# dordanino12/unet-convlstm

Hardware: AMD Instinct MI355X
Metric: training frames/sec, Moving-MNIST 64x64 seq-20 (higher is better)
Workload: dtype bf16; 1 GPU; TemporalUNetDualView(base_ch=64, use_skip_lstm=True) train step, 64x64 seq-20, per-GPU batch 32, AdamW+clip; global_batch=32, seq_len=20, parallelism=dp1

## Files before the change

include/uclstm.h:

```cpp
#ifndef UCLSTM_H
#define UCLSTM_H

#include <stdint.h>

#ifdef __cplusplus
extern "C" {
#endif

#define UCLSTM_ABI_VERSION 16

#define UCLSTM_OK            0
#define UCLSTM_E_BADARG     -1
#define UCLSTM_E_LAUNCH     -2
#define UCLSTM_E_NODEVICE   -3

#define UCLSTM_ACT_TYPE_BF16 0
#define UCLSTM_ACT_TYPE_F16  1


typedef struct {
    const void* ptr;
    int32_t C;
    int32_t Hs, Ws;
    int32_t offY, offX;
} uclstm_src;

typedef struct {
    void* ptr;
    int32_t n_begin, n_end;
    int32_t C, c_off;
    int32_t Hd, Wd;
    int32_t scale, oy, ox;
} uclstm_seg;

#define UCLSTM_EPI_STORE 0
#define UCLSTM_EPI_LSTM  1
#define UCLSTM_EPI_ATOMIC 2

typedef struct {
    int32_t n_img, H, W, groups;
    int32_t ktap, scale, pad;
    int32_t nsrc;
    uclstm_src src[2];
    const void* wp;
    int32_t N, Ktot;
    const float* bias;
    const float* col_scale;
    const float* col_shift;
    int32_t relu;
    int32_t epi;
    int32_t nseg;
    uclstm_seg seg[4];
    float* stats;
    int32_t Hd_p;
    const float* c_prev;
    float* c_out;
    void* h_out;
    void* gates_out;
    const float* pre_add;
    float* acc_out;
    int32_t acc_ld;
    int32_t ksplit;
    int64_t acc_slab;
} uclstm_igemm_desc;

int32_t uclstm_igemm_tiles_per_group(int32_t n_img, int32_t H, int32_t W, int32_t groups, int32_t N);

int32_t uclstm_igemm_fwd(const uclstm_igemm_desc* d, void* stream);
int32_t uclstm_igemm_fwd_shape(const uclstm_igemm_desc* desc);
int32_t uclstm_igemm_ksplit_used(int32_t Ktot, int32_t ktap, int32_t ksplit);

int32_t uclstm_igemm_fwd_group(const uclstm_igemm_desc* descs, int32_t n, void* stream);
int32_t uclstm_igemm_fwd_group_blocks(const uclstm_igemm_desc* descs, int32_t n);

int32_t uclstm_igemm_fwd_group_tap(const uclstm_igemm_desc* descs, int32_t n, void* stream);
int32_t uclstm_igemm_fwd_group_tap_blocks(const uclstm_igemm_desc* descs, int32_t n);

typedef struct {
    int32_t n_img, H, W;
    int32_t ktap, scale, pad;
    int32_t nsrc;
    uclstm_src src[2];
    int32_t N, Ktot;
    int32_t nseg;
    uclstm_seg seg[4];
    float* dwp;
    int32_t splits;
    int32_t accumulate;
    int32_t overlapped;
    int32_t reserved_;
    int64_t slab;
} uclstm_wgrad_desc;
int32_t uclstm_igemm_wgrad(const uclstm_wgrad_desc* d, void* stream);
int32_t uclstm_igemm_wgrad_splits(const uclstm_wgrad_desc* d);
int32_t uclstm_igemm_wgrad_shape(const uclstm_wgrad_desc* d);

#define UCLSTM_NMODE_IDENTITY 0
#define UCLSTM_NMODE_LSTM     1
#define UCLSTM_NMODE_TAPMAJOR 2
#define UCLSTM_KMODE_IDENTITY 0
#define UCLSTM_KMODE_GATES    1
#define UCLSTM_KMODE_IM2COL   2

typedef struct {
    int32_t N, Ktot;
    int32_t taps, nsrc;
    int32_t kseg[2], cvalid[2], choff[2];
    int32_t n_mode, n_valid, n_cp;
    int32_t k_mode, k_hdp, k_hd;
    int32_t tap_flip;
    int64_t stride_n, stride_k, stride_tap, stride_ntap;
} uclstm_pack_desc;

int32_t uclstm_pack_weights(const uclstm_pack_desc* d, const float* w, void* wp, void* stream);
typedef struct {
    uclstm_pack_desc d;
    const float* w;
    void* wp;
    int32_t block0, nblocks, gx, family;
    uint32_t div[15];
    int32_t pad_;
} uclstm_pack_job;
int32_t uclstm_pack_job_init(uclstm_pack_job* job , const uclstm_pack_desc* d, const float* w, void* wp, int32_t block0);
int32_t uclstm_pack_weights_batched(const uclstm_pack_job* jobs_dev ,
                                    int32_t njobs, int32_t family, int32_t total_blocks, void* stream);

int32_t uclstm_unpack_wgrad(const uclstm_pack_desc* d, const float* dwp, int32_t nslab ,
                            int64_t slab , float* grad, int32_t accumulate, void* stream);
int32_t uclstm_unpack_wgrad_ordered_groups(const uclstm_pack_desc* d, int32_t nslab);
int32_t uclstm_unpack_wgrad_ordered(const uclstm_pack_desc* d, const float* dwp, int32_t nslab, int64_t slab, float* scratch,
                                    float* grad, int32_t accumulate, void* stream);
int32_t uclstm_pack_bias(const uclstm_pack_desc* d, const float* b, float* bp, void* stream);

int32_t uclstm_bn_finalize(float* stats, int32_t groups, int32_t tiles_per_group, int32_t Cp, int32_t C,
                           int64_t count_per_group, const float* gamma, const float* beta,
                           float* running_mean, float* running_var, float momentum, float eps,
                           float* scale, float* shift, float* mean, float* rstd, void* stream);
int32_t uclstm_bn_stats_fwd(float* stats, int32_t groups, int32_t tiles_per_group, int32_t Cp, int32_t C, int64_t count_per_group,
                            const float* gamma, const float* beta, float eps, float* scale, float* shift, float* mean, float* rstd,
                            void* stream);
int32_t uclstm_bn_running_stats(const float* stats, int32_t groups, int32_t tiles_per_group, int32_t Cp, int32_t C,
                                int64_t count_per_group, float* running_mean, float* running_var, float momentum, void* stream);

int32_t uclstm_bn_stats_partial(const float* stats, int32_t groups, int32_t tiles_per_group, int32_t Cp, double* sums64, void* stream);
int32_t uclstm_bn_stats_from_sums(const double* sums64, int64_t world_count_per_group, float* stats, int32_t groups,
                                  int32_t tiles_per_group, int32_t Cp, int32_t C, const float* gamma, const float* beta, float eps,
                                  float* scale, float* shift, float* mean, float* rstd, void* stream);
int32_t uclstm_bn_bwd_sums_stage(const float* sums, double* sums64, int64_t n, void* stream);
int32_t uclstm_bn_bwd_sums_finish(const double* sums64, double inv_world, float* sums_dz, int64_t n, void* stream);

int32_t uclstm_bn_apply_relu(const void* z, void* a, const float* scale, const float* shift,
                             int64_t pixels, int64_t pixels_per_group, int32_t Cp, void* stream);
int64_t uclstm_bn_bwd_reduce_rows(int64_t pixels, int64_t pixels_per_group);
int32_t uclstm_bn_bwd_reduce(const void* z, const void* da, const float* scale, const float* shift,
                             const float* mean, const float* rstd, float* partials, float* sums,
                             int64_t pixels, int64_t pixels_per_group, int32_t Cp, void* stream);
int32_t uclstm_bn_bwd_apply(const void* z, const void* da, const float* scale, const float* shift,
                            const float* mean, const float* rstd, const float* sums, void* dz,
                            int64_t pixels, int64_t pixels_per_group, int32_t Cp, void* stream);

int64_t uclstm_bn_pool_bwd_rows(int64_t n_img, int32_t H, int32_t W, int32_t Cp, int32_t groups);
int32_t uclstm_bn_apply_relu_pool(const void* z, void* a, void* p, const float* scale, const float* shift, int64_t n_img, int32_t H,
                                  int32_t W, int32_t Cp, int32_t groups, void* stream);
int32_t uclstm_bn_pool_bwd_reduce(const void* z, const void* dskip, const void* dp, const float* scale, const float* shift,
                                  const float* mean, const float* rstd, float* partials, float* sums, int64_t n_img, int32_t H,
                                  int32_t W, int32_t Cp, int32_t groups, void* stream);
int32_t uclstm_bn_pool_bwd_apply(const void* z, const void* dskip, const void* dp, const float* scale, const float* shift,
                                 const float* mean, const float* rstd, const float* sums, void* dz, int64_t n_img, int32_t H,
                                 int32_t W, int32_t Cp, int32_t groups, void* stream);

int32_t uclstm_bn_head_fwd(const void* z, const float* scale, const float* shift, const float* w, const float* b, float* y,
                           int64_t pixels, int64_t pixels_per_group, int32_t Cp, int32_t C, void* stream);
int32_t uclstm_bn_head_bwd_reduce(const void* z, const float* dy, const float* scale, const float* shift, const float* mean,
                                  const float* rstd, const float* w, float* partials, float* sums, float* dw, float* db,
                                  int64_t pixels, int64_t pixels_per_group, int32_t Cp, int32_t C, void* stream);
int32_t uclstm_bn_head_bwd_apply(const void* z, const float* dy, const float* scale, const float* shift, const float* mean,
                                 const float* rstd, const float* sums, const float* w, void* dz, int64_t pixels,
                                 int64_t pixels_per_group, int32_t Cp, int32_t C, void* stream);

int32_t uclstm_bn_head_bwd_reduce_ordered(const void* z, const float* dy, const float* scale, const float* shift, const float* mean,
                                          const float* rstd, const float* w, float* partials, float* head_partials, float* sums,
                                          float* dw, float* db, int64_t pixels, int64_t pixels_per_group, int32_t Cp, int32_t C,
                                          int32_t act_type, void* stream);

int32_t uclstm_bn_bwd_param_grads(const float* sums, int32_t groups, int32_t Cp, int32_t C, float* dgamma, float* dbeta,
                                  int32_t accumulate, void* stream);

int32_t uclstm_maxpool2_fwd(const void* a, void* p, int32_t n_img, int32_t H, int32_t W, int32_t Cp, void* stream);
int32_t uclstm_maxpool2_bwd(const void* a, const void* dp, const void* add, void* da, int32_t n_img, int32_t H, int32_t W, int32_t Cp,
                            void* stream);

int32_t uclstm_splitk_finish(const float* pre, int32_t nslab, int64_t slab, int32_t ld, const float* bias, const float* col_scale,
                             const float* col_shift, int32_t relu, void* out, int64_t pixels, int32_t C, void* stream);

int32_t uclstm_lstm_bwd_pointwise(const void* gates, const float* c_prev, const float* c_new,
                                  const void* dh_a, const void* dh_b, int32_t dh_b_is_f32 ,
                                  int32_t dh_b_nslab , int64_t dh_b_slab ,
                                  float* dc_io, int32_t dc_is_zero, void* dgates, int64_t pixels, int32_t Hd_p, void* stream);
int32_t uclstm_lstm_fwd_pointwise(float* pre, int32_t nslab ,
                                  int64_t slab ,
                                  int32_t clear ,
                                  const float* pre_add ,
                                  const float* bias, const float* c_prev, float* c_out, void* h_out,
                                  void* gates_out, int64_t pixels, int32_t Hd_p, void* stream);
typedef struct {
    float* pre;
    const float* pre_add;
    const float* bias;
    const float* c_prev;
    float* c_out;
    void* h_out;
    void* gates_out;
    int64_t slab;
    int64_t pixels;
    int32_t nslab, clear, Hd_p, reserved_;
} uclstm_lstm_fwd_pw_args;
int32_t uclstm_lstm_fwd_pointwise_group(const uclstm_lstm_fwd_pw_args* args, int32_t n, void* stream);

int32_t uclstm_nchw_to_nhwc(const float* x, void* out, int32_t n_img, int32_t C, int32_t Cp, int32_t H, int32_t W,
                            int32_t inner, int64_t inner_stride, int64_t outer_stride, void* stream);
int32_t uclstm_nhwc_to_nchw(const void* a, float* out, int32_t n_img, int32_t C, int32_t Cp, int32_t H, int32_t W, void* stream);
int32_t uclstm_nchw_grad_to_nhwc(const float* g, void* out, int32_t n_img, int32_t C, int32_t Cp, int32_t H, int32_t W, void* stream);
int32_t uclstm_im2col3x3_first(const float* x, void* out, int32_t n_img, int32_t C, int32_t Kp, int32_t H, int32_t W,
                               int32_t inner, int64_t inner_stride, int64_t outer_stride, void* stream);
int32_t uclstm_nchw_to_nhwc_f32(const float* x, float* out, int32_t n_img, int32_t C, int32_t Cp, int32_t H, int32_t W, void* stream);
int32_t uclstm_nhwc_to_nchw_f32(const float* a, float* out, int32_t n_img, int32_t C, int32_t Cp, int32_t H, int32_t W, void* stream);

int32_t uclstm_outconv_fwd(const void* a, const float* w, const float* b, float* y,
                           int64_t n_img, int32_t HW, int32_t Cp, int32_t C, int32_t Co, void* stream);
int32_t uclstm_outconv_bwd(const void* a, const float* w, const float* dy, void* da, float* dw, float* db,
                           int64_t n_img, int32_t HW, int32_t Cp, int32_t C, int32_t Co, void* stream);

int64_t uclstm_outconv_bwd_ordered_rows(int64_t n_img, int32_t HW);
int32_t uclstm_outconv_bwd_ordered(const void* a, const float* w, const float* dy, void* da, float* partials, float* dw, float* db,
                                   int32_t accumulate, int64_t n_img, int32_t HW, int32_t Cp, int32_t C, int32_t Co,
                                   int32_t act_type, void* stream);

int32_t uclstm_attention_fwd(const void* x, const float* w, void* out, float* att, float* desc, int32_t* argmax, int32_t n_img,
                             int32_t H, int32_t W, int32_t Cp, int32_t C, int32_t k, void* stream);
int32_t uclstm_attention_bwd(const void* x, const void* dout, const float* w, const float* att, const float* desc,
                             const int32_t* argmax, void* dx, float* dw, int32_t dw_accumulate, float* scratch, int32_t n_img,
                             int32_t H, int32_t W, int32_t Cp, int32_t C, int32_t k, void* stream);

int32_t uclstm_colsum(const void* a, float* out, int64_t pixels, int32_t Cp, void* stream);
int64_t uclstm_colsum_ordered_rows(int64_t pixels, int32_t Cp);
int32_t uclstm_colsum_ordered(const void* a, float* partials, float* out, int64_t pixels, int32_t Cp, int32_t accumulate,
                              int32_t act_type, void* stream);
int32_t uclstm_ordered_sum_f32(const float* partials, int32_t rows, int32_t cols, float* out, int32_t accumulate, void* stream);
int32_t uclstm_ordered_sum_f64(const double* partials, int32_t rows, int32_t cols, double* out, int32_t accumulate, void* stream);

int32_t uclstm_loss_fwd(const float* y_pred, const float* y, const float* mask, double* sums,
                        int64_t planes, int32_t H, int32_t W, void* stream);
int64_t uclstm_loss_fwd_ordered_rows(int64_t planes, int32_t H, int32_t W);
int32_t uclstm_loss_fwd_ordered(const float* y_pred, const float* y, const float* mask, double* partials, double* sums,
                                int32_t accumulate, int64_t planes, int32_t H, int32_t W, void* stream);
int32_t uclstm_loss_bwd(const float* y_pred, const float* y, const float* mask, const float* coefs,
                        float* grad, int64_t planes, int32_t H, int32_t W, void* stream);

#define UCLSTM_LOSS_POINT_L1 0
#define UCLSTM_LOSS_POINT_L2 1
#define UCLSTM_LOSS_POINT_HUBER 2
typedef struct uclstm_loss_spec {
    int32_t point;
    int32_t weight_power;
    float delta;
    float weight_gain;
    int32_t grad_term;
    int32_t reserved[3];
} uclstm_loss_spec;
int32_t uclstm_loss_spec_fwd(const uclstm_loss_spec* spec, const float* y_pred, const float* y, const float* mask, double* sums,
                             int64_t planes, int32_t H, int32_t W, void* stream);
int32_t uclstm_loss_spec_fwd_ordered(const uclstm_loss_spec* spec, const float* y_pred, const float* y, const float* mask,
                                     double* partials, double* sums, int32_t accumulate, int64_t planes, int32_t H, int32_t W,
                                     void* stream);
int32_t uclstm_loss_spec_bwd(const uclstm_loss_spec* spec, const float* y_pred, const float* y, const float* mask,
                             const float* coefs, float* grad, int64_t planes, int32_t H, int32_t W, void* stream);
int32_t uclstm_loss_spec_fwd_bc(const uclstm_loss_spec* spec, const float* y_pred, const float* y, const float* mask, double* sums,
                                int64_t planes, int32_t H, int32_t W, int32_t mask_div, void* stream);
int32_t uclstm_loss_spec_fwd_ordered_bc(const uclstm_loss_spec* spec, const float* y_pred, const float* y, const float* mask,
                                        double* partials, double* sums, int32_t accumulate, int64_t planes, int32_t H, int32_t W,
                                        int32_t mask_div, void* stream);
int32_t uclstm_loss_spec_bwd_bc(const uclstm_loss_spec* spec, const float* y_pred, const float* y, const float* mask,
                                const float* coefs, float* grad, int64_t planes, int32_t H, int32_t W, int32_t mask_div, void* stream);

int32_t uclstm_sumsq(const float* g, int64_t n, double* out , void* stream);
int64_t uclstm_sumsq_ordered_rows(int64_t n);
int32_t uclstm_sumsq_ordered(const float* g, int64_t n, double* partials, double* out, int32_t accumulate, void* stream);
int32_t uclstm_adamw_step(float* p, float* m, float* v, const float* g, int64_t n, const double* sumsq, float max_norm,
                          float lr, float beta1, float beta2, float eps, float weight_decay, int32_t step, void* stream);

int32_t uclstm_adamw_step_dev(float* p, float* m, float* v, const float* g, int64_t n, const double* sumsq, float* hyper, void* stream);

int32_t uclstm_adamw_step_groups(float* p, float* m, float* v, const float* g, int64_t n, const double* sumsq,
                                 const int64_t* runs, int32_t n_runs, float* hyper, int32_t n_groups,
                                 const float* scale_state, void* stream);

int32_t uclstm_adamw_step_scaled(float* p, float* m, float* v, const float* g, int64_t n, const double* sumsq, float max_norm,
                                 float lr, float beta1, float beta2, float eps, float weight_decay, const float* scale_state,
                                 void* stream);
int32_t uclstm_loss_scale_update(float* scale_state, const double* sumsq, float growth, float backoff, int32_t interval,
                                 void* stream);

int32_t uclstm_dataset_transform(const float* x_raw, const float* y_raw, float* x, float* y, float* mask, int64_t n_frames,
                                 int32_t C, int32_t HW, float norm_const, float min_vel, float max_vel, int32_t clip,
                                 float y_scale, float trans_min, float trans_max, void* stream);
int32_t uclstm_dataset_gather_transform(const float* x_all, const float* y_all, const int64_t* idx, int64_t n_seq, int64_t n_out,
                                        int32_t T, int32_t C, int32_t HW, float* x, float* y, float* mask, int32_t transform,
                                        float norm_const, float min_vel, float max_vel, int32_t clip, float y_scale,
                                        float trans_min, float trans_max, void* stream);
int32_t uclstm_dataset_gather_augment(const float* x_all, const float* y_all, const int64_t* idx, const int32_t* aug,
        int64_t n_seq, int64_t n_out, int32_t T_src, int32_t T_out, int32_t C, int32_t Hs, int32_t Ws, int32_t Ho, int32_t Wo,
        int32_t flags, float* x, float* y, float* mask, int32_t transform, float norm_const, float min_vel, float max_vel, int32_t clip,
        float y_scale, float trans_min, float trans_max, void* stream);
int32_t uclstm_plane_d4(const float* src, float* dst, int64_t n_planes, int32_t H, int32_t W, int32_t code, int32_t accumulate,
                        float scale, void* stream);
#define UCLSTM_VEC_MAX 4
typedef struct {
    float min_vel, max_vel, y_scale, trans_min, trans_max;
} uclstm_target_consts;
int32_t uclstm_dataset_gather_vec(const float* x_all, const float* y_all, const int64_t* idx, const int32_t* aug ,
        int64_t n_seq, int64_t n_out, int32_t T_src, int32_t T_out, int32_t C, int32_t Cy, int32_t Hs, int32_t Ws, int32_t Ho, int32_t Wo,
        int32_t flags, const int8_t* chan_map ,
        float* x, float* y, float* mask, int32_t transform, float norm_const, int32_t clip,
        const uclstm_target_consts* consts , void* stream);
int32_t uclstm_plane_d4_vec(const float* src, float* dst, int64_t n_frames, int32_t Cy, int32_t H, int32_t W, int32_t code,
        const int8_t* chan_map , const float* offset , int32_t accumulate, float scale, void* stream);
int32_t uclstm_sprites_render(const uint8_t* bank, int32_t n_glyph, int32_t gh, int32_t gw, const int32_t* table, int64_t n_out,
                              int32_t D, int32_t T, int32_t C, int32_t H, int32_t W, float v_scale, float* x, float* y,
                              float* mask, float* raw, void* stream);
int32_t uclstm_metric_sums(const float* y_pred, const float* y, const float* mask, double* sums, int64_t n, float y_scale,
                           float trans_min, float trans_max, void* stream);

int64_t uclstm_metric_sums_ordered_rows(int64_t n);
int32_t uclstm_metric_sums_ordered(const float* y_pred, const float* y, const float* mask, double* partials, double* sums,
                                   int32_t accumulate, int64_t n, float y_scale, float trans_min, float trans_max, void* stream);
int64_t uclstm_metric_sums_vec_rows(int64_t n_frames, int32_t Cy, int32_t HW);
int32_t uclstm_metric_sums_vec(const float* y_pred, const float* y, const float* mask, double* partials, double* sums,
                               int32_t accumulate, int64_t n_frames, int32_t Cy, int32_t HW, int32_t transform,
                               const uclstm_target_consts* consts , void* stream);

#define UCLSTM_EVAL_ROW         16
#define UCLSTM_EVAL_NONE         0
#define UCLSTM_EVAL_ASINH        1
#define UCLSTM_EVAL_SIGNED_LOG   2
typedef struct {
    const float* y_pred; int64_t pred_stride_b, pred_stride_t;
    const float* y;      int64_t y_stride_b, y_stride_t;
    const float* mask;   int64_t mask_stride_b, mask_stride_t;
    int32_t B, T;
    int64_t P;
    int32_t transform;
    float y_scale, trans_min, trans_max;
    double* table;
    int32_t bins, n_edges;
    double hist_lo, hist_hi, err_lo, err_hi;
    double dig_lo, dig_w;
    uint64_t* hist;
    uint64_t* dig_count;
    float* scatter;
    uint64_t seed;
    int32_t K, reserved_;
} uclstm_eval_desc;
int32_t uclstm_eval_stats(const uclstm_eval_desc* d, void* stream);
int64_t uclstm_eval_stats_rows(int64_t P, int64_t frames);

#define UCLSTM_EVAL_VROW        16
typedef struct {
    const float* y_pred; int64_t pred_stride_b, pred_stride_t;
    const float* y;      int64_t y_stride_b, y_stride_t;
    const float* mask;   int64_t mask_stride_b, mask_stride_t;
    int32_t B, T, Cy;
    int32_t transform;
    int64_t HW;
    uclstm_target_consts consts[UCLSTM_VEC_MAX];
    double hist_lo[UCLSTM_VEC_MAX], hist_hi[UCLSTM_VEC_MAX], err_lo[UCLSTM_VEC_MAX], err_hi[UCLSTM_VEC_MAX];
    double dig_lo[UCLSTM_VEC_MAX], dig_w[UCLSTM_VEC_MAX];
    int32_t bins, n_edges, K, dir_bins;
    uint64_t seed;
    int32_t w_chan, h_chan;
    int32_t w_sign, h_sign;
    double speed_hi, epe_hi, min_speed;
    double* table;
    uint64_t* hist;
    uint64_t* dig_count;
    float* scatter;
    double* vtable;
    uint64_t* vhist;
    uint64_t* dir_hist;
} uclstm_eval_vec_desc;
int32_t uclstm_eval_stats_vec(const uclstm_eval_vec_desc* d, void* stream);

#define UCLSTM_SELECT_MAX_SLOTS 8
#define UCLSTM_SELECT_BINS 2048
#define UCLSTM_SELECT_SIGNED 0
#define UCLSTM_SELECT_ABS 1
#define UCLSTM_SELECT_WS_COUNT 0
#define UCLSTM_SELECT_WS_NAN 1
#define UCLSTM_SELECT_WS_FLAGS 2
#define UCLSTM_SELECT_WS_PREFIX 8
#define UCLSTM_SELECT_WS_RANK 16
#define UCLSTM_SELECT_WS_LEADER 24
#define UCLSTM_SELECT_WS_HIST 32
#define UCLSTM_SELECT_WS_WORDS (UCLSTM_SELECT_WS_HIST + UCLSTM_SELECT_MAX_SLOTS * UCLSTM_SELECT_BINS)
typedef struct {
    void* workspace;
    int32_t n_slots;
    uint32_t abs_mask;
    int32_t phase;
    uint32_t magic;
} uclstm_select_state;
int64_t uclstm_select_workspace_bytes(void);
int32_t uclstm_select_begin(uclstm_select_state* state, void* workspace, const int64_t* ranks, const int32_t* kinds, int32_t n_slots,
                            void* stream);
int32_t uclstm_select_accumulate(uclstm_select_state* state, int32_t pass, const float* v, int64_t n, void* stream);
int32_t uclstm_select_narrow(uclstm_select_state* state, int32_t pass, void* stream);
int32_t uclstm_select_finish(uclstm_select_state* state, float* out_values, uint64_t* out_info, void* stream);
#define UCLSTM_EXTREMES_MIN_KEY 0
#define UCLSTM_EXTREMES_MAX_KEY 1
#define UCLSTM_EXTREMES_NAN 2
#define UCLSTM_EXTREMES_NONZERO 3
#define UCLSTM_EXTREMES_COUNT 4
#define UCLSTM_EXTREMES_WORDS 8
int32_t uclstm_dataset_extremes_begin(uint64_t* out, void* stream);
int32_t uclstm_dataset_extremes(const float* v, int64_t n, uint64_t* out, void* stream);

int32_t uclstm_stream_spin(int32_t microseconds, void* stream);


int32_t uclstm_im2col7x7s2_first(const float* x, void* out, int32_t n_img, int32_t C, int32_t Kp, int32_t H, int32_t W,
                                 int32_t inner, int64_t inner_stride, int64_t outer_stride, void* stream);
int32_t uclstm_maxpool3s2_fwd(const void* a, void* p, int32_t n_img, int32_t H, int32_t W, int32_t Cp, void* stream);
int32_t uclstm_bn_add_relu(const void* z, const float* scale, const float* shift, const void* r, const float* rscale,
                           const float* rshift, void* a, int64_t pixels, int32_t Cp, void* stream);
int32_t uclstm_upsample2_fwd(const void* a, void* out, int32_t n_img, int32_t H, int32_t W, int32_t Cp, void* stream);
int32_t uclstm_upsample2_bwd(const void* dout, void* da, int32_t n_img, int32_t H, int32_t W, int32_t Cp, void* stream);
int32_t uclstm_head3x3_fwd(const void* a, const float* w, const float* b, float* y, int64_t n_img, int32_t H, int32_t W, int32_t Cp,
                           int32_t C, int32_t Co, void* stream);
int32_t uclstm_head3x3_bwd(const void* a, const float* w, const float* dy, void* da, float* dw, float* db, int64_t n_img, int32_t H,
                           int32_t W, int32_t Cp, int32_t C, int32_t Co, void* stream);
int64_t uclstm_head3x3_bwd_ordered_rows(int64_t n_img, int32_t H, int32_t W);
int32_t uclstm_head3x3_bwd_ordered(const void* a, const float* w, const float* dy, void* da, float* partials, float* dw, float* db,
                                   int32_t accumulate, int64_t n_img, int32_t H, int32_t W, int32_t Cp, int32_t C, int32_t Co,
                                   int32_t act_type, void* stream);

int32_t uclstm_maxpool3s2_bwd(const void* a, const void* dp, const void* dskip, void* da, int32_t n_img, int32_t H, int32_t W,
                              int32_t Cp, void* stream);
int64_t uclstm_bn_add_relu_bwd_rows(int64_t pixels);
int32_t uclstm_bn_add_relu_bwd_reduce(const void* z, const float* scale, const float* shift, const float* mean, const float* rstd,
                                      const void* r, const float* rscale, const float* rshift, const float* rmean,
                                      const float* rrstd, const void* da, float* partials, float* sums, float* rsums,
                                      int64_t pixels, int32_t Cp, void* stream);
int32_t uclstm_bn_add_relu_bwd_apply(const void* z, const float* scale, const float* shift, const float* mean, const float* rstd,
                                     const float* sums, const void* r, const float* rscale, const float* rshift,
                                     const float* rmean, const float* rrstd, const float* rsums, const void* da, void* dz,
                                     void* dr, int64_t pixels, int32_t Cp, void* stream);

#define UCLSTM_F16_TWIN(fn) __typeof__(fn) fn##_f16;
UCLSTM_F16_TWIN(uclstm_igemm_fwd)
UCLSTM_F16_TWIN(uclstm_igemm_fwd_group)
UCLSTM_F16_TWIN(uclstm_igemm_wgrad)
UCLSTM_F16_TWIN(uclstm_pack_weights)
UCLSTM_F16_TWIN(uclstm_pack_weights_batched)
UCLSTM_F16_TWIN(uclstm_bn_apply_relu)
UCLSTM_F16_TWIN(uclstm_bn_bwd_reduce)
UCLSTM_F16_TWIN(uclstm_bn_bwd_apply)
UCLSTM_F16_TWIN(uclstm_bn_apply_relu_pool)
UCLSTM_F16_TWIN(uclstm_bn_pool_bwd_reduce)
UCLSTM_F16_TWIN(uclstm_bn_pool_bwd_apply)
UCLSTM_F16_TWIN(uclstm_bn_head_fwd)
UCLSTM_F16_TWIN(uclstm_bn_head_bwd_reduce)
UCLSTM_F16_TWIN(uclstm_bn_head_bwd_apply)
UCLSTM_F16_TWIN(uclstm_maxpool2_fwd)
UCLSTM_F16_TWIN(uclstm_maxpool2_bwd)
UCLSTM_F16_TWIN(uclstm_lstm_bwd_pointwise)
UCLSTM_F16_TWIN(uclstm_lstm_fwd_pointwise)
UCLSTM_F16_TWIN(uclstm_lstm_fwd_pointwise_group)
UCLSTM_F16_TWIN(uclstm_splitk_finish)
UCLSTM_F16_TWIN(uclstm_nchw_to_nhwc)
UCLSTM_F16_TWIN(uclstm_nhwc_to_nchw)
UCLSTM_F16_TWIN(uclstm_nchw_grad_to_nhwc)
UCLSTM_F16_TWIN(uclstm_im2col3x3_first)
UCLSTM_F16_TWIN(uclstm_outconv_fwd)
UCLSTM_F16_TWIN(uclstm_outconv_bwd)
UCLSTM_F16_TWIN(uclstm_colsum)
UCLSTM_F16_TWIN(uclstm_attention_fwd)
UCLSTM_F16_TWIN(uclstm_attention_bwd)
#define UCLSTM_RESNET_F16_TWINS(TWIN) \
    TWIN(uclstm_im2col7x7s2_first) TWIN(uclstm_maxpool3s2_fwd) TWIN(uclstm_bn_add_relu) TWIN(uclstm_upsample2_fwd) \
    TWIN(uclstm_upsample2_bwd) TWIN(uclstm_head3x3_fwd) TWIN(uclstm_head3x3_bwd)
UCLSTM_RESNET_F16_TWINS(UCLSTM_F16_TWIN)
#define UCLSTM_RESNET_BWD_F16_TWINS(TWIN) \
    TWIN(uclstm_maxpool3s2_bwd) TWIN(uclstm_bn_add_relu_bwd_reduce) TWIN(uclstm_bn_add_relu_bwd_apply)
UCLSTM_RESNET_BWD_F16_TWINS(UCLSTM_F16_TWIN)
#define UCLSTM_TAP_GROUP_F16_TWINS(TWIN) TWIN(uclstm_igemm_fwd_group_tap)
UCLSTM_TAP_GROUP_F16_TWINS(UCLSTM_F16_TWIN)

int32_t uclstm_abi_version(void);
const char* uclstm_build_arch(void);
const char* uclstm_source_hash(void);
const char* uclstm_last_error_string(void);

#ifdef __cplusplus
}
#endif
#endif
```

unet-convlstm_amd/_lib.py:

```python
from __future__ import annotations

import ctypes as C
import os
import re

import torch

HERE = os.path.dirname(os.path.abspath(__file__))
LIB_PATH = os.environ.get("UCLSTM_LIB") or os.path.join(HERE, "libuclstm.so")
HEADER_PATH = os.path.join(HERE, "..", "include", "uclstm.h")

ABI_VERSION = 16
EPI_STORE, EPI_LSTM, EPI_ATOMIC = 0, 1, 2
NMODE_IDENTITY, NMODE_LSTM, NMODE_TAPMAJOR = 0, 1, 2
KMODE_IDENTITY, KMODE_GATES, KMODE_IM2COL = 0, 1, 2
ACT_TYPE_BF16, ACT_TYPE_F16 = 0, 1

_ERRORS = {-1: "bad argument (shape/alignment/null contract)", -2: "kernel launch failed", -3: "no gfx950 device"}


class UclstmError(RuntimeError):
    pass


class Src(C.Structure):
    _fields_ = [("ptr", C.c_void_p), ("C", C.c_int32), ("Hs", C.c_int32), ("Ws", C.c_int32),
                ("offY", C.c_int32), ("offX", C.c_int32)]


class Seg(C.Structure):
    _fields_ = [("ptr", C.c_void_p), ("n_begin", C.c_int32), ("n_end", C.c_int32), ("C", C.c_int32),
                ("c_off", C.c_int32), ("Hd", C.c_int32), ("Wd", C.c_int32), ("scale", C.c_int32),
                ("oy", C.c_int32), ("ox", C.c_int32)]


class IgemmDesc(C.Structure):
    _fields_ = [("n_img", C.c_int32), ("H", C.c_int32), ("W", C.c_int32), ("groups", C.c_int32),
                ("ktap", C.c_int32), ("scale", C.c_int32), ("pad", C.c_int32), ("nsrc", C.c_int32),
                ("src", Src * 2),
                ("wp", C.c_void_p), ("N", C.c_int32), ("Ktot", C.c_int32),
                ("bias", C.c_void_p), ("col_scale", C.c_void_p), ("col_shift", C.c_void_p),
                ("relu", C.c_int32), ("epi", C.c_int32),
                ("nseg", C.c_int32), ("seg", Seg * 4),
                ("stats", C.c_void_p),
                ("Hd_p", C.c_int32), ("c_prev", C.c_void_p), ("c_out", C.c_void_p), ("h_out", C.c_void_p),
                ("gates_out", C.c_void_p), ("pre_add", C.c_void_p),
                ("acc_out", C.c_void_p), ("acc_ld", C.c_int32), ("ksplit", C.c_int32), ("acc_slab", C.c_int64)]


class WgradDesc(C.Structure):
    _fields_ = [("n_img", C.c_int32), ("H", C.c_int32), ("W", C.c_int32),
                ("ktap", C.c_int32), ("scale", C.c_int32), ("pad", C.c_int32), ("nsrc", C.c_int32),
                ("src", Src * 2),
                ("N", C.c_int32), ("Ktot", C.c_int32),
                ("nseg", C.c_int32), ("seg", Seg * 4),
                ("dwp", C.c_void_p), ("splits", C.c_int32), ("accumulate", C.c_int32), ("overlapped", C.c_int32), ("reserved_", C.c_int32),
                ("slab", C.c_int64)]


class LstmFwdPwArgs(C.Structure):
    _fields_ = [("pre", C.c_void_p), ("pre_add", C.c_void_p), ("bias", C.c_void_p), ("c_prev", C.c_void_p), ("c_out", C.c_void_p),
                ("h_out", C.c_void_p), ("gates_out", C.c_void_p), ("slab", C.c_int64), ("pixels", C.c_int64),
                ("nslab", C.c_int32), ("clear", C.c_int32), ("Hd_p", C.c_int32), ("reserved_", C.c_int32)]


class PackDesc(C.Structure):
    _fields_ = [("N", C.c_int32), ("Ktot", C.c_int32), ("taps", C.c_int32), ("nsrc", C.c_int32),
                ("kseg", C.c_int32 * 2), ("cvalid", C.c_int32 * 2), ("choff", C.c_int32 * 2),
                ("n_mode", C.c_int32), ("n_valid", C.c_int32), ("n_cp", C.c_int32),
                ("k_mode", C.c_int32), ("k_hdp", C.c_int32), ("k_hd", C.c_int32),
                ("tap_flip", C.c_int32),
                ("stride_n", C.c_int64), ("stride_k", C.c_int64), ("stride_tap", C.c_int64),
                ("stride_ntap", C.c_int64)]


class PackJob(C.Structure):
    _fields_ = [("d", PackDesc), ("w", C.c_void_p), ("wp", C.c_void_p),
                ("block0", C.c_int32), ("nblocks", C.c_int32), ("gx", C.c_int32), ("family", C.c_int32),
                ("div", C.c_uint32 * 15), ("pad_", C.c_int32)]


class EvalDesc(C.Structure):
    _fields_ = [("y_pred", C.c_void_p), ("pred_stride_b", C.c_int64), ("pred_stride_t", C.c_int64),
                ("y", C.c_void_p), ("y_stride_b", C.c_int64), ("y_stride_t", C.c_int64),
                ("mask", C.c_void_p), ("mask_stride_b", C.c_int64), ("mask_stride_t", C.c_int64),
                ("B", C.c_int32), ("T", C.c_int32), ("P", C.c_int64),
                ("transform", C.c_int32), ("y_scale", C.c_float), ("trans_min", C.c_float), ("trans_max", C.c_float),
                ("table", C.c_void_p), ("bins", C.c_int32), ("n_edges", C.c_int32),
                ("hist_lo", C.c_double), ("hist_hi", C.c_double), ("err_lo", C.c_double), ("err_hi", C.c_double),
                ("dig_lo", C.c_double), ("dig_w", C.c_double),
                ("hist", C.c_void_p), ("dig_count", C.c_void_p), ("scatter", C.c_void_p),
                ("seed", C.c_uint64), ("K", C.c_int32), ("reserved_", C.c_int32)]


class LossSpecDesc(C.Structure):
    _fields_ = [("point", C.c_int32), ("weight_power", C.c_int32), ("delta", C.c_float), ("weight_gain", C.c_float),
                ("grad_term", C.c_int32), ("reserved_", C.c_int32 * 3)]


class SelectState(C.Structure):
    _fields_ = [("workspace", C.c_void_p), ("n_slots", C.c_int32), ("abs_mask", C.c_uint32), ("phase", C.c_int32), ("magic", C.c_uint32)]


class TargetConsts(C.Structure):
    _fields_ = [("min_vel", C.c_float), ("max_vel", C.c_float), ("y_scale", C.c_float), ("trans_min", C.c_float), ("trans_max", C.c_float)]


class EvalVecDesc(C.Structure):
    _fields_ = [("y_pred", C.c_void_p), ("pred_stride_b", C.c_int64), ("pred_stride_t", C.c_int64),
                ("y", C.c_void_p), ("y_stride_b", C.c_int64), ("y_stride_t", C.c_int64),
                ("mask", C.c_void_p), ("mask_stride_b", C.c_int64), ("mask_stride_t", C.c_int64),
                ("B", C.c_int32), ("T", C.c_int32), ("Cy", C.c_int32), ("transform", C.c_int32), ("HW", C.c_int64),
                ("consts", TargetConsts * 4),
                ("hist_lo", C.c_double * 4), ("hist_hi", C.c_double * 4), ("err_lo", C.c_double * 4), ("err_hi", C.c_double * 4),
                ("dig_lo", C.c_double * 4), ("dig_w", C.c_double * 4),
                ("bins", C.c_int32), ("n_edges", C.c_int32), ("K", C.c_int32), ("dir_bins", C.c_int32),
                ("seed", C.c_uint64),
                ("w_chan", C.c_int32), ("h_chan", C.c_int32), ("w_sign", C.c_int32), ("h_sign", C.c_int32),
                ("speed_hi", C.c_double), ("epe_hi", C.c_double), ("min_speed", C.c_double),
                ("table", C.c_void_p), ("hist", C.c_void_p), ("dig_count", C.c_void_p), ("scatter", C.c_void_p),
                ("vtable", C.c_void_p), ("vhist", C.c_void_p), ("dir_hist", C.c_void_p)]


LOSS_POINT_L1, LOSS_POINT_L2, LOSS_POINT_HUBER = 0, 1, 2
VEC_MAX = 4
SELECT_MAX_SLOTS, SELECT_BINS, SELECT_SIGNED, SELECT_ABS = 8, 2048, 0, 1
SELECT_WS_COUNT, SELECT_WS_NAN, SELECT_WS_FLAGS, SELECT_WS_PREFIX, SELECT_WS_RANK, SELECT_WS_LEADER, SELECT_WS_HIST = 0, 1, 2, 8, 16, 24, 32
EXTREMES_MIN_KEY, EXTREMES_MAX_KEY, EXTREMES_NAN, EXTREMES_NONZERO, EXTREMES_COUNT, EXTREMES_WORDS = 0, 1, 2, 3, 4, 8
EVAL_ROW = 16
EVAL_VROW = 16
EVAL_NONE, EVAL_ASINH, EVAL_SIGNED_LOG = 0, 1, 2

_P, _I, _L, _F = C.c_void_p, C.c_int32, C.c_int64, C.c_float

_PROTOS = {
    "uclstm_igemm_tiles_per_group": [_I, _I, _I, _I, _I],
    "uclstm_igemm_fwd": [C.POINTER(IgemmDesc), _P],
    "uclstm_igemm_fwd_shape": [_P],
    "uclstm_igemm_ksplit_used": [_I, _I, _I],
    "uclstm_igemm_fwd_group": [C.POINTER(IgemmDesc), _I, _P],
    "uclstm_igemm_fwd_group_blocks": [C.POINTER(IgemmDesc), _I],
    "uclstm_igemm_fwd_group_tap": [C.POINTER(IgemmDesc), _I, _P],
    "uclstm_igemm_fwd_group_tap_blocks": [C.POINTER(IgemmDesc), _I],
    "uclstm_igemm_wgrad": [C.POINTER(WgradDesc), _P],
    "uclstm_igemm_wgrad_splits": [C.POINTER(WgradDesc)],
    "uclstm_igemm_wgrad_shape": [C.POINTER(WgradDesc)],
    "uclstm_pack_weights": [C.POINTER(PackDesc), _P, _P, _P],
    "uclstm_pack_job_init": [C.POINTER(PackJob), C.POINTER(PackDesc), _P, _P, _I],
    "uclstm_pack_weights_batched": [_P, _I, _I, _I, _P],
    "uclstm_unpack_wgrad": [C.POINTER(PackDesc), _P, _I, _L, _P, _I, _P],
    "uclstm_unpack_wgrad_ordered_groups": [C.POINTER(PackDesc), _I],
    "uclstm_unpack_wgrad_ordered": [C.POINTER(PackDesc), _P, _I, _L, _P, _P, _I, _P],
    "uclstm_pack_bias": [C.POINTER(PackDesc), _P, _P, _P],
    "uclstm_bn_finalize": [_P, _I, _I, _I, _I, _L, _P, _P, _P, _P, _F, _F, _P, _P, _P, _P, _P],
    "uclstm_bn_stats_fwd": [_P, _I, _I, _I, _I, _L, _P, _P, _F, _P, _P, _P, _P, _P],
    "uclstm_bn_running_stats": [_P, _I, _I, _I, _I, _L, _P, _P, _F, _P],
    "uclstm_bn_stats_partial": [_P, _I, _I, _I, _P, _P],
    "uclstm_bn_stats_from_sums": [_P, _L, _P, _I, _I, _I, _I, _P, _P, _F, _P, _P, _P, _P, _P],
    "uclstm_bn_bwd_sums_stage": [_P, _P, _L, _P],
    "uclstm_bn_bwd_sums_finish": [_P, C.c_double, _P, _L, _P],
    "uclstm_bn_apply_relu": [_P, _P, _P, _P, _L, _L, _I, _P],
    "uclstm_bn_bwd_reduce_rows": [_L, _L],
    "uclstm_bn_bwd_reduce": [_P, _P, _P, _P, _P, _P, _P, _P, _L, _L, _I, _P],
    "uclstm_bn_bwd_apply": [_P, _P, _P, _P, _P, _P, _P, _P, _L, _L, _I, _P],
    "uclstm_bn_pool_bwd_rows": [_L, _I, _I, _I, _I],
    "uclstm_bn_apply_relu_pool": [_P, _P, _P, _P, _P, _L, _I, _I, _I, _I, _P],
    "uclstm_bn_pool_bwd_reduce": [_P, _P, _P, _P, _P, _P, _P, _P, _P, _L, _I, _I, _I, _I, _P],
    "uclstm_bn_pool_bwd_apply": [_P, _P, _P, _P, _P, _P, _P, _P, _P, _L, _I, _I, _I, _I, _P],
    "uclstm_bn_head_fwd": [_P, _P, _P, _P, _P, _P, _L, _L, _I, _I, _P],
    "uclstm_bn_head_bwd_reduce": [_P, _P, _P, _P, _P, _P, _P, _P, _P, _P, _P, _L, _L, _I, _I, _P],
    "uclstm_bn_head_bwd_reduce_ordered": [_P, _P, _P, _P, _P, _P, _P, _P, _P, _P, _P, _P, _L, _L, _I, _I, _I, _P],
    "uclstm_bn_head_bwd_apply": [_P, _P, _P, _P, _P, _P, _P, _P, _P, _L, _L, _I, _I, _P],
    "uclstm_bn_bwd_param_grads": [_P, _I, _I, _I, _P, _P, _I, _P],
    "uclstm_maxpool2_fwd": [_P, _P, _I, _I, _I, _I, _P],
    "uclstm_maxpool2_bwd": [_P, _P, _P, _P, _I, _I, _I, _I, _P],
    "uclstm_lstm_bwd_pointwise": [_P, _P, _P, _P, _P, _I, _I, _L, _P, _I, _P, _L, _I, _P],
    "uclstm_lstm_fwd_pointwise": [_P, _I, _L, _I, _P, _P, _P, _P, _P, _P, _L, _I, _P],
    "uclstm_lstm_fwd_pointwise_group": [C.POINTER(LstmFwdPwArgs), _I, _P],
    "uclstm_splitk_finish": [_P, _I, _L, _I, _P, _P, _P, _I, _P, _L, _I, _P],
    "uclstm_nchw_to_nhwc": [_P, _P, _I, _I, _I, _I, _I, _I, _L, _L, _P],
    "uclstm_nhwc_to_nchw": [_P, _P, _I, _I, _I, _I, _I, _P],
    "uclstm_nchw_grad_to_nhwc": [_P, _P, _I, _I, _I, _I, _I, _P],
    "uclstm_im2col3x3_first": [_P, _P, _I, _I, _I, _I, _I, _I, _L, _L, _P],
    "uclstm_nchw_to_nhwc_f32": [_P, _P, _I, _I, _I, _I, _I, _P],
    "uclstm_nhwc_to_nchw_f32": [_P, _P, _I, _I, _I, _I, _I, _P],
    "uclstm_outconv_fwd": [_P, _P, _P, _P, _L, _I, _I, _I, _I, _P],
    "uclstm_outconv_bwd": [_P, _P, _P, _P, _P, _P, _L, _I, _I, _I, _I, _P],
    "uclstm_outconv_bwd_ordered_rows": [_L, _I],
    "uclstm_outconv_bwd_ordered": [_P, _P, _P, _P, _P, _P, _P, _I, _L, _I, _I, _I, _I, _I, _P],
    "uclstm_im2col7x7s2_first": [_P, _P, _I, _I, _I, _I, _I, _I, _L, _L, _P],
    "uclstm_maxpool3s2_fwd": [_P, _P, _I, _I, _I, _I, _P],
    "uclstm_bn_add_relu": [_P, _P, _P, _P, _P, _P, _P, _L, _I, _P],
    "uclstm_upsample2_fwd": [_P, _P, _I, _I, _I, _I, _P],
    "uclstm_upsample2_bwd": [_P, _P, _I, _I, _I, _I, _P],
    "uclstm_head3x3_fwd": [_P, _P, _P, _P, _L, _I, _I, _I, _I, _I, _P],
    "uclstm_head3x3_bwd": [_P, _P, _P, _P, _P, _P, _L, _I, _I, _I, _I, _I, _P],
    "uclstm_head3x3_bwd_ordered_rows": [_L, _I, _I],
    "uclstm_head3x3_bwd_ordered": [_P, _P, _P, _P, _P, _P, _P, _I, _L, _I, _I, _I, _I, _I, _I, _P],
    "uclstm_maxpool3s2_bwd": [_P, _P, _P, _P, _I, _I, _I, _I, _P],
    "uclstm_bn_add_relu_bwd_rows": [_L],
    "uclstm_bn_add_relu_bwd_reduce": [_P] * 14 + [_L, _I, _P],
    "uclstm_bn_add_relu_bwd_apply": [_P] * 15 + [_L, _I, _P],
    "uclstm_colsum": [_P, _P, _L, _I, _P],
    "uclstm_colsum_ordered_rows": [_L, _I],
    "uclstm_colsum_ordered": [_P, _P, _P, _L, _I, _I, _I, _P],
    "uclstm_ordered_sum_f32": [_P, _I, _I, _P, _I, _P],
    "uclstm_ordered_sum_f64": [_P, _I, _I, _P, _I, _P],
    "uclstm_attention_fwd": [_P, _P, _P, _P, _P, _P, _I, _I, _I, _I, _I, _I, _P],
    "uclstm_attention_bwd": [_P, _P, _P, _P, _P, _P, _P, _P, _I, _P, _I, _I, _I, _I, _I, _I, _P],
    "uclstm_loss_fwd": [_P, _P, _P, _P, _L, _I, _I, _P],
    "uclstm_loss_fwd_ordered_rows": [_L, _I, _I],
    "uclstm_loss_fwd_ordered": [_P, _P, _P, _P, _P, _I, _L, _I, _I, _P],
    "uclstm_loss_bwd": [_P, _P, _P, _P, _P, _L, _I, _I, _P],
    "uclstm_loss_spec_fwd": [C.POINTER(LossSpecDesc), _P, _P, _P, _P, _L, _I, _I, _P],
    "uclstm_loss_spec_fwd_ordered": [C.POINTER(LossSpecDesc), _P, _P, _P, _P, _P, _I, _L, _I, _I, _P],
    "uclstm_loss_spec_bwd": [C.POINTER(LossSpecDesc), _P, _P, _P, _P, _P, _L, _I, _I, _P],
    "uclstm_loss_spec_fwd_bc": [C.POINTER(LossSpecDesc), _P, _P, _P, _P, _L, _I, _I, _I, _P],
    "uclstm_loss_spec_fwd_ordered_bc": [C.POINTER(LossSpecDesc), _P, _P, _P, _P, _P, _I, _L, _I, _I, _I, _P],
    "uclstm_loss_spec_bwd_bc": [C.POINTER(LossSpecDesc), _P, _P, _P, _P, _P, _L, _I, _I, _I, _P],
    "uclstm_sumsq": [_P, _L, _P, _P],
    "uclstm_sumsq_ordered_rows": [_L],
    "uclstm_sumsq_ordered": [_P, _L, _P, _P, _I, _P],
    "uclstm_adamw_step": [_P, _P, _P, _P, _L, _P, _F, _F, _F, _F, _F, _F, _I, _P],
    "uclstm_adamw_step_dev": [_P, _P, _P, _P, _L, _P, _P, _P],
    "uclstm_adamw_step_groups": [_P, _P, _P, _P, _L, _P, _P, _I, _P, _I, _P, _P],
    "uclstm_adamw_step_scaled": [_P, _P, _P, _P, _L, _P, _F, _F, _F, _F, _F, _F, _P, _P],
    "uclstm_loss_scale_update": [_P, _P, _F, _F, _I, _P],
    "uclstm_dataset_transform": [_P, _P, _P, _P, _P, _L, _I, _I, _F, _F, _F, _I, _F, _F, _F, _P],
    "uclstm_dataset_gather_transform": [_P, _P, _P, _L, _L, _I, _I, _I, _P, _P, _P, _I, _F, _F, _F, _I, _F, _F, _F, _P],
    "uclstm_dataset_gather_augment": [_P, _P, _P, _P, _L, _L, _I, _I, _I, _I, _I, _I, _I, _I, _P, _P, _P, _I, _F, _F, _F, _I, _F, _F, _F, _P],
    "uclstm_plane_d4": [_P, _P, _L, _I, _I, _I, _I, _F, _P],
    "uclstm_dataset_gather_vec": [_P, _P, _P, _P, _L, _L, _I, _I, _I, _I, _I, _I, _I, _I, _I, _P, _P, _P, _P, _I, _F, _I, C.POINTER(TargetConsts), _P],
    "uclstm_plane_d4_vec": [_P, _P, _L, _I, _I, _I, _I, _P, _P, _I, _F, _P],
    "uclstm_sprites_render": [_P, _I, _I, _I, _P, _L, _I, _I, _I, _I, _I, _F, _P, _P, _P, _P, _P],
    "uclstm_metric_sums": [_P, _P, _P, _P, _L, _F, _F, _F, _P],
    "uclstm_metric_sums_ordered_rows": [_L],
    "uclstm_metric_sums_ordered": [_P, _P, _P, _P, _P, _I, _L, _F, _F, _F, _P],
    "uclstm_metric_sums_vec_rows": [_L, _I, _I],
    "uclstm_metric_sums_vec": [_P, _P, _P, _P, _P, _I, _L, _I, _I, _I, C.POINTER(TargetConsts), _P],
    "uclstm_eval_stats": [C.POINTER(EvalDesc), _P],
    "uclstm_eval_stats_rows": [_L, _L],
    "uclstm_eval_stats_vec": [C.POINTER(EvalVecDesc), _P],
    "uclstm_select_workspace_bytes": [],
    "uclstm_select_begin": [C.POINTER(SelectState), _P, C.POINTER(C.c_int64), C.POINTER(C.c_int32), _I, _P],
    "uclstm_select_accumulate": [C.POINTER(SelectState), _I, _P, _L, _P],
    "uclstm_select_narrow": [C.POINTER(SelectState), _I, _P],
    "uclstm_select_finish": [C.POINTER(SelectState), _P, _P, _P],
    "uclstm_dataset_extremes_begin": [_P, _P],
    "uclstm_dataset_extremes": [_P, _L, _P, _P],
    "uclstm_stream_spin": [_I, _P],
    "uclstm_abi_version": [],
    "uclstm_build_arch": [],
    "uclstm_source_hash": [],
    "uclstm_last_error_string": [],
}
_RESTYPES = {"uclstm_build_arch": C.c_char_p, "uclstm_source_hash": C.c_char_p, "uclstm_last_error_string": C.c_char_p, "uclstm_bn_bwd_reduce_rows": C.c_int64, "uclstm_bn_pool_bwd_rows": C.c_int64,
             "uclstm_eval_stats_rows": C.c_int64, "uclstm_colsum_ordered_rows": C.c_int64, "uclstm_outconv_bwd_ordered_rows": C.c_int64, "uclstm_head3x3_bwd_ordered_rows": C.c_int64,
             "uclstm_loss_fwd_ordered_rows": C.c_int64, "uclstm_sumsq_ordered_rows": C.c_int64, "uclstm_metric_sums_ordered_rows": C.c_int64, "uclstm_metric_sums_vec_rows": C.c_int64,
             "uclstm_bn_add_relu_bwd_rows": C.c_int64, "uclstm_select_workspace_bytes": C.c_int64}


F16_TWINS = ['uclstm_igemm_fwd', 'uclstm_igemm_fwd_group', 'uclstm_igemm_wgrad', 'uclstm_pack_weights', 'uclstm_pack_weights_batched', 'uclstm_bn_apply_relu', 'uclstm_bn_bwd_reduce', 'uclstm_bn_bwd_apply', 'uclstm_bn_apply_relu_pool', 'uclstm_bn_pool_bwd_reduce', 'uclstm_bn_pool_bwd_apply', 'uclstm_bn_head_fwd', 'uclstm_bn_head_bwd_reduce', 'uclstm_bn_head_bwd_apply', 'uclstm_maxpool2_fwd', 'uclstm_maxpool2_bwd', 'uclstm_lstm_bwd_pointwise', 'uclstm_lstm_fwd_pointwise', 'uclstm_lstm_fwd_pointwise_group', 'uclstm_splitk_finish', 'uclstm_nchw_to_nhwc', 'uclstm_nhwc_to_nchw', 'uclstm_nchw_grad_to_nhwc', 'uclstm_im2col3x3_first', 'uclstm_outconv_fwd', 'uclstm_outconv_bwd', 'uclstm_colsum', 'uclstm_attention_fwd', 'uclstm_attention_bwd']
RESNET_F16_TWINS = ['uclstm_im2col7x7s2_first', 'uclstm_maxpool3s2_fwd', 'uclstm_bn_add_relu', 'uclstm_upsample2_fwd', 'uclstm_upsample2_bwd',
                    'uclstm_head3x3_fwd', 'uclstm_head3x3_bwd']
RESNET_BWD_F16_TWINS = ['uclstm_maxpool3s2_bwd', 'uclstm_bn_add_relu_bwd_reduce', 'uclstm_bn_add_relu_bwd_apply']
TAP_GROUP_F16_TWINS = ['uclstm_igemm_fwd_group_tap']
_ALL_F16_TWINS = frozenset(F16_TWINS) | frozenset(RESNET_F16_TWINS) | frozenset(RESNET_BWD_F16_TWINS) | frozenset(TAP_GROUP_F16_TWINS)


def header_symbols() -> list[str]:
    with open(HEADER_PATH) as f:
        text = f.read()
    names = set(re.findall(r"\b(uclstm_[a-z0-9_]+)\s*\(", text))
    names |= {n + "_f16" for n in re.findall(r"^UCLSTM_F16_TWIN\((uclstm_[a-z0-9_]+)\)", text, re.M)}
    return sorted(names)


def _load() -> C.CDLL:
    if not os.path.exists(LIB_PATH):
        raise UclstmError(
            f"{LIB_PATH} is missing: build it with `python unet-convlstm_amd/build.py` "
            "(hipcc --offload-arch=gfx950). There is no CPU or PyTorch fallback for this package.")
    lib = C.CDLL(LIB_PATH)
    for name, argtypes in list(_PROTOS.items()):
        for sym in ([name, name + "_f16"] if name in _ALL_F16_TWINS else [name]):
            try:
                fn = getattr(lib, sym)
            except AttributeError as e:
                raise UclstmError(f"{LIB_PATH} does not export {sym}; rebuild the library") from e
            fn.argtypes = argtypes
            fn.restype = _RESTYPES.get(name, C.c_int32)
    if lib.uclstm_abi_version() != ABI_VERSION:
        raise UclstmError("libuclstm.so ABI version mismatch; rebuild the library")
    if not os.environ.get("UCLSTM_LIB"):
        from . import build as _build
        built, tree = lib.uclstm_source_hash().decode(), _build.source_hash()
        if built != tree:
            raise UclstmError(f"{LIB_PATH} was built from other sources than this tree (library {built[:16]}, tree {tree[:16]}): "
                              "run `python unet-convlstm_amd/build.py`")
    return lib


lib = _load()


class _F16Kernels:

    def __getattr__(self, name):
        fn = getattr(lib, name + "_f16" if name in _ALL_F16_TWINS else name)
        setattr(self, name, fn)
        return fn


lib16 = _F16Kernels()


def kernels(dtype):
    if dtype == torch.bfloat16:
        return lib
    if dtype == torch.float16:
        return lib16
    raise UclstmError(f"activations must be torch.bfloat16 or torch.float16, got {dtype}")


def act_type(dtype) -> int:
    if dtype == torch.bfloat16:
        return ACT_TYPE_BF16
    if dtype == torch.float16:
        return ACT_TYPE_F16
    raise UclstmError(f"activations must be torch.bfloat16 or torch.float16, got {dtype}")


def check(rc: int, what: str) -> None:
    if rc != 0:
        detail = f" [{lib.uclstm_last_error_string().decode()}]" if rc == -2 else ""
        raise UclstmError(f"{what}: {_ERRORS.get(rc, 'error')} (code {rc}){detail}")
```

unet-convlstm_amd/csrc/igemm_wgrad.hip:

```cpp
#include "common.h"
#include <cstdlib>

namespace {

constexpr int TN = 128;
constexpr int TC = 128;
constexpr int TP = 64;
constexpr int PITCH = 256;
constexpr int TILE_BYTES = TP * PITCH;
constexpr int STAGE_BYTES = 2 * TILE_BYTES;
constexpr int SMEM_BYTES = 2 * STAGE_BYTES;

__device__ uint4 g_wzero_page[2];

struct WDerived {
    int kseg0, kseg1;
    int n_kt, n_nt;
    long M;
    long chunk;
    int kt_per_tap;
    FastDiv dHW, dW, dPerTap;
};

typedef __attribute__((address_space(3))) short4v* lds_s4p;
typedef __attribute__((address_space(3))) void* lds_ptr;
typedef const __attribute__((address_space(1))) void* gbl_ptr;

__device__ __forceinline__ act16x8 tr_frag(const unsigned char* p) {
    const short4v lo = __builtin_amdgcn_ds_read_tr16_b64_v4i16((lds_s4p)(p));
    const short4v hi = __builtin_amdgcn_ds_read_tr16_b64_v4i16((lds_s4p)(p + 16 * PITCH));
    typedef __attribute__((ext_vector_type(8))) short short8v;
    const short8v v = {lo.x, lo.y, lo.z, lo.w, hi.x, hi.y, hi.z, hi.w};
    return __builtin_bit_cast(act16x8, v);
}

__device__ __forceinline__ uint64_t select_addr(uint64_t a, uint32_t ok, uint64_t zero) {
    uint32_t lo = (uint32_t)a, hi = (uint32_t)(a >> 32);
    asm volatile("v_cmp_ne_u32 vcc, 0, %2\n\tv_cndmask_b32 %0, %3, %0, vcc\n\tv_cndmask_b32 %1, %4, %1, vcc"
                 : "+v"(lo), "+v"(hi)
                 : "v"(ok), "v"((uint32_t)zero), "v"((uint32_t)(zero >> 32))
                 : "vcc");
    return ((uint64_t)hi << 32) | lo;
}

template <bool PLAIN>
__global__ __launch_bounds__(256, 2) void igemm_wgrad_kernel(const uclstm_wgrad_desc d, const WDerived dv) {
    extern __shared__ __attribute__((aligned(16))) unsigned char smem[];

    const int tid = threadIdx.x;
    const int lane = tid & 63;
    const int wave = tid >> 6;
    const int wc = wave >> 1;
    const int wk = wave & 1;
    const int l15 = lane & 15;
    const int lq = lane >> 4;

    const int per_split = dv.n_kt * dv.n_nt;
    const int lid = xcd_remap(blockIdx.x, per_split * d.splits);
    const int sp = lid / per_split;
    const int rr = lid - sp * per_split;
    const int kt = rr / dv.n_nt;
    const int nt = rr - kt * dv.n_nt;
    const int n0 = nt * TN;
    const int kbase = kt * TC;

    const long m_begin = (long)sp * dv.chunk;
    if (m_begin >= dv.M) return;
    const long m_end = min(dv.M, m_begin + dv.chunk);
    const int nsteps = (int)((m_end - m_begin + TP - 1) / TP);
    const int HW = d.H * d.W;
    const uint64_t zero_addr = (uint64_t)(const void*)g_wzero_page;

    const int lrow0 = 4 * wave + lq;
    const int cp = l15;
    const int sc = 2 * ((cp >> 1) ^ (lrow0 & 7)) + (cp & 1);

    const int ny = n0 + sc * 8;
    int sgi = -1;
#pragma unroll
    for (int i = 0; i < 4; ++i)
        if (i < d.nseg && ny < d.N && ny >= d.seg[i].n_begin && ny < d.seg[i].n_end) sgi = i;
    const uclstm_seg G = d.seg[sgi < 0 ? 0 : sgi];
    const uint32_t yok = sgi >= 0 ? 1u : 0u;
    const int ycol = G.c_off + (ny - G.n_begin);

    const int kx = kbase + sc * 8;
    const int xtap = (int)fdiv((uint32_t)kx, dv.dPerTap);
    const int kr = kx - xtap * (dv.kseg0 + dv.kseg1);
    const int xs_ = kr >= dv.kseg0 ? 1 : 0;
    const int xc = xs_ ? kr - dv.kseg0 : kr;
    const uclstm_src S = d.src[(xs_ < d.nsrc) ? xs_ : 0];
    const uint32_t xok = (kx < d.Ktot && xs_ < d.nsrc && xc < S.C) ? 1u : 0u;
    const int tdy = xtap / d.ktap;
    const int ddy = tdy - d.pad - S.offY;
    const int ddx = (xtap - tdy * d.ktap) - d.pad - S.offX;

    const int ystride = G.C, xstride = S.C;
    const int xshift = (ddy * S.Ws + ddx) * S.C + xc;

    f32x4 acc[4][4];
#pragma unroll
    for (int a = 0; a < 4; ++a)
#pragma unroll
        for (int b = 0; b < 4; ++b) acc[a][b] = (f32x4){0.f, 0.f, 0.f, 0.f};

    int lstep = 0;
    auto issue_loads = [&](int buf) {
        unsigned char* Y = smem + buf * STAGE_BYTES;
        unsigned char* X = Y + TILE_BYTES;
        const uint32_t mb = (uint32_t)(m_begin + (long)lstep * TP);
#pragma unroll
        for (int j = 0; j < 4; ++j) {
            const uint32_t m = mb + lrow0 + 16 * j;
            const uint32_t inr = (long)m < m_end ? 1u : 0u;
            const uint32_t img = fdiv(m, dv.dHW);
            const uint32_t rem = m - img * (uint32_t)HW;
            const int y = (int)fdiv(rem, dv.dW);
            const int x = (int)rem - y * d.W;
            uint64_t ay, ax;
            uint32_t oky = yok & inr, okx = xok & inr;
            if constexpr (PLAIN) {
                ay = (uint64_t)G.ptr + (uint64_t)((long)(int)(m * (uint32_t)ystride + (uint32_t)ycol) * 2);
                ax = (uint64_t)S.ptr + (uint64_t)((long)((int)(m * (uint32_t)xstride) + xshift) * 2);
                okx &= ((unsigned)(y + ddy) < (unsigned)S.Hs && (unsigned)(x + ddx) < (unsigned)S.Ws) ? 1u : 0u;
            } else {
                const int yd = y * G.scale + G.oy, xd = x * G.scale + G.ox;
                oky &= ((unsigned)yd < (unsigned)G.Hd && (unsigned)xd < (unsigned)G.Wd) ? 1u : 0u;
                ay = (uint64_t)G.ptr + (uint64_t)((long)((((int)img * G.Hd + yd) * G.Wd + xd) * G.C + ycol) * 2);
                const int ys = y * d.scale + ddy, xs = x * d.scale + ddx;
                okx &= ((unsigned)ys < (unsigned)S.Hs && (unsigned)xs < (unsigned)S.Ws) ? 1u : 0u;
                ax = (uint64_t)S.ptr + (uint64_t)((long)((((int)img * S.Hs + ys) * S.Ws + xs) * S.C + xc) * 2);
            }
            ay = select_addr(ay, oky, zero_addr);
            ax = select_addr(ax, okx, zero_addr);
            const int ldso = (16 * j + 4 * wave) * PITCH;
            __builtin_amdgcn_global_load_lds((gbl_ptr)ay, (lds_ptr)(Y + ldso), 16, 0, 0);
            __builtin_amdgcn_global_load_lds((gbl_ptr)ax, (lds_ptr)(X + ldso), 16, 0, 0);
        }
        ++lstep;
    };

    const int trow = 4 * lq + (l15 >> 2);
    const int rsw = trow & 7;
    const int tr_base = trow * PITCH + (l15 & 3) * 8;
    int goffy[4], goffx[4];
#pragma unroll
    for (int a = 0; a < 4; ++a) {
        goffy[a] = (((wc * 4 + a) ^ rsw) << 5) + tr_base;
        goffx[a] = (((wk * 4 + a) ^ rsw) << 5) + tr_base;
    }
    auto compute = [&](int buf) {
        const unsigned char* Y = smem + buf * STAGE_BYTES;
        const unsigned char* X = Y + TILE_BYTES;
#pragma unroll
        for (int ks = 0; ks < 2; ++ks) {
            act16x8 yf[4], xf[4];
#pragma unroll
            for (int a = 0; a < 4; ++a) yf[a] = tr_frag(Y + ks * 32 * PITCH + goffy[a]);
#pragma unroll
            for (int b = 0; b < 4; ++b) xf[b] = tr_frag(X + ks * 32 * PITCH + goffx[b]);
#pragma unroll
            for (int a = 0; a < 4; ++a)
#pragma unroll
                for (int b = 0; b < 4; ++b)
                    acc[a][b] = UCLSTM_MFMA_16x16x32(yf[a], xf[b], acc[a][b], 0, 0, 0);
        }
    };

    issue_loads(0);
    __syncthreads();
    for (int step = 0; step < nsteps; ++step) {
        if (step + 1 < nsteps) issue_loads((step + 1) & 1);
        compute(step & 1);
        __syncthreads();
    }

    constexpr int AP = TC + 4;
    float* At = (float*)smem;
#pragma unroll
    for (int half = 0; half < 2; ++half) {
        if (wc == half) {
#pragma unroll
            for (int a = 0; a < 4; ++a)
#pragma unroll
                for (int b = 0; b < 4; ++b)
#pragma unroll
                    for (int r = 0; r < 4; ++r) At[(a * 16 + lq * 4 + r) * AP + wk * 64 + b * 16 + l15] = acc[a][b][r];
        }
        __syncthreads();
        const int k = kbase + (tid & 127);
        if (k < d.Ktot) {
            for (int pr = tid >> 7; pr < 64; pr += 2) {
                const int n = n0 + half * 64 + pr;
                if (n < d.N)
                    {
                    float* dst = d.dwp + (long)sp * d.slab + (long)n * d.Ktot + k;
                    if (d.slab > 0) *dst = At[pr * AP + (tid & 127)];
                    else __hip_atomic_fetch_add(dst, At[pr * AP + (tid & 127)], __ATOMIC_RELAXED, __HIP_MEMORY_SCOPE_AGENT);
                }
            }
        }
        __syncthreads();
    }
}


struct P2 {
    int lw, lh;
    uint32_t ybytes;
    uint32_t xbytes[2];
    uint32_t xbias[2];
};

constexpr int PLANE = TP * 128;
constexpr uint32_t OOB = 0x80000000u;

template <int WN>
struct WShape {
    static constexpr int WNR = WN == 2 ? 2 : 1;
    static constexpr int WK = 4 / WNR;
    static constexpr int XP = WN == 3 ? 3 : WK;
    static constexpr int NB = WN == 3 ? 3 : 4;
    static constexpr int WCOLS = 16 * NB;
    static constexpr int TN_ = 64 * WNR, TC_ = 64 * XP;
    static constexpr int NPL = WNR + XP;
    static constexpr int STAGE = NPL * PLANE;
    static constexpr int SMEM = 2 * STAGE;
    static constexpr int NI = 2 * NPL;
};

__device__ __forceinline__ act16x8 tr_frag128(const unsigned char* p) {
    const short4v lo = __builtin_amdgcn_ds_read_tr16_b64_v4i16((lds_s4p)(p));
    const short4v hi = __builtin_amdgcn_ds_read_tr16_b64_v4i16((lds_s4p)(p + 16 * 128));
    typedef __attribute__((ext_vector_type(8))) short short8v;
    const short8v v = {lo.x, lo.y, lo.z, lo.w, hi.x, hi.y, hi.z, hi.w};
    return __builtin_bit_cast(act16x8, v);
}

template <int WN, int NSRC>
__global__ __launch_bounds__(256, 2) void igemm_wgrad_p2_kernel(const uclstm_wgrad_desc d, const WDerived dv, const P2 p2) {
#if defined(__HIP_DEVICE_COMPILE__)
    using SH = WShape<WN>;
    constexpr int WK = SH::WK;
    extern __shared__ __attribute__((aligned(16))) unsigned char smem[];

    const int tid = threadIdx.x;
    const int lane = tid & 63;
    const int wave = __builtin_amdgcn_readfirstlane(tid >> 6);
    const int wc = wave / WK;
    const int wk = wave % WK;
    const int l15 = lane & 15;
    const int lq = lane >> 4;

    const int per_split = dv.n_kt * dv.n_nt;
    const int lid = xcd_remap(blockIdx.x, per_split * d.splits);
    const int sp = lid / per_split;
    const int rr = lid - sp * per_split;
    int nt, kts;
    grouped_tile(rr, dv.n_nt, dv.n_kt, 8, nt, kts);
    int kt = kts;
    if (dv.kt_per_tap > 0) {
        const int ntaps = d.ktap * d.ktap;
        const int cg = kts / ntaps;
        kt = (kts - cg * ntaps) * dv.kt_per_tap + cg;
    }
    const int n0 = nt * SH::TN_;
    const int kbase = kt * SH::TC_;

    const long m_begin = (long)sp * dv.chunk;
    if (m_begin >= dv.M) return;
    const long m_end = min(dv.M, m_begin + dv.chunk);
    const int nsteps = (int)((m_end - m_begin) / TP);

    const uclstm_seg G = d.seg[0];
    const __amdgpu_buffer_rsrc_t rsy = __builtin_amdgcn_make_buffer_rsrc((void*)G.ptr, 0, p2.ybytes, 0x00020000);
    const __amdgpu_buffer_rsrc_t rsx0 =
        __builtin_amdgcn_make_buffer_rsrc((void*)((const unsigned char*)d.src[0].ptr - p2.xbias[0]), 0, p2.xbytes[0], 0x00020000);
    const __amdgpu_buffer_rsrc_t rsx1 =
        NSRC > 1 ? __builtin_amdgcn_make_buffer_rsrc((void*)((const unsigned char*)d.src[1].ptr - p2.xbias[1]), 0, p2.xbytes[1], 0x00020000)
                 : rsx0;

    const int lrow = lane >> 3;
    const int cp = lane & 7;
    const int sc = 2 * ((cp >> 1) ^ ((lrow >> 1) & 3)) + (cp & 1);
    const int Wm = d.W - 1, Hm = d.H - 1;
    const int kseg = dv.kseg0 + dv.kseg1;

    uint32_t voff[SH::NI];
    uint32_t kxj[2 * SH::XP], kyj[2 * SH::XP];
    int xsrc[SH::XP];
#pragma unroll
    for (int j = 0; j < SH::NI; ++j) {
        const int pl = j >> 1;
        const int r = 8 * (4 * (j & 1) + wave) + lrow;
        if (pl < SH::WNR) {
            const int ny = n0 + pl * 64 + sc * 8;
            const bool yok = ny < d.N && ny >= G.n_begin && ny < G.n_end;
            voff[j] = yok ? (uint32_t)(2 * (r * G.C + G.c_off + (ny - G.n_begin))) : OOB;
        } else {
            const int xp = pl - SH::WNR;
            const int k0 = kbase + xp * 64;
            const int xtap = (int)fdiv((uint32_t)k0, dv.dPerTap);
            const int kr = k0 - xtap * kseg;
            const int xs_ = (NSRC > 1 && kr >= dv.kseg0) ? 1 : 0;
            const int xc = (xs_ ? kr - dv.kseg0 : kr) + sc * 8;
            const uclstm_src S = d.src[xs_];
            const bool xok = k0 < d.Ktot && xc < S.C;
            const int tdy = xtap / d.ktap;
            const int ddy = tdy - d.pad;
            const int ddx = (xtap - tdy * d.ktap) - d.pad;
            const int badx = ddx < 0 ? 0 : (ddx > 0 ? Wm : -1);
            const int bady = ddy < 0 ? 0 : (ddy > 0 ? Hm : -1);
            if ((j & 1) == 0) xsrc[xp] = xs_;
            voff[j] = xok ? (uint32_t)(2 * (r * S.C + (ddy * S.Ws + ddx) * S.C + xc) + (int)p2.xbias[xs_]) : OOB;
            const int jj = j - 2 * SH::WNR;
            if (badx < 0) kxj[jj] = 0xffffffffu;
            else if (d.W >= 64) kxj[jj] = (uint32_t)(badx - r);
            else kxj[jj] = ((r & Wm) == badx) ? 0u : 0xffffffffu;
            kyj[jj] = bady < 0 ? 0xffffffffu : (uint32_t)((bady - (r >> p2.lw)) & Hm);
        }
    }
    const uint32_t ystep = (uint32_t)(2 * G.C), x0step = (uint32_t)(2 * d.src[0].C), x1step = (uint32_t)(2 * d.src[NSRC - 1].C);

    constexpr int NB = SH::NB;
    f32x4 acc[4][NB];
#pragma unroll
    for (int a = 0; a < 4; ++a)
#pragma unroll
        for (int b = 0; b < NB; ++b) acc[a][b] = (f32x4){0.f, 0.f, 0.f, 0.f};

    uint32_t mb = (uint32_t)m_begin;
    auto issue_loads = [&](int buf) {
        unsigned char* St = smem + buf * SH::STAGE;
        const uint32_t sy = (mb >> p2.lw) & (uint32_t)Hm;
        const uint32_t sx = mb & (uint32_t)Wm;
        const uint32_t ysoff = mb * ystep, x0soff = mb * x0step, x1soff = mb * x1step;
#pragma unroll
        for (int j = 0; j < SH::NI; ++j) {
            lds_ptr dst = (lds_ptr)(St + (j >> 1) * PLANE + (4 * (j & 1) + wave) * 1024);
            if (j < 2 * SH::WNR) {
                __builtin_amdgcn_raw_ptr_buffer_load_lds(rsy, dst, 16, voff[j], ysoff, 0, 0);
            } else {
                const int jj = j - 2 * SH::WNR;
                const bool ok = (sx != kxj[jj]) & (sy != kyj[jj]);
                const uint32_t off = ok ? voff[j] : OOB;
                if (NSRC == 1 || xsrc[jj >> 1] == 0) __builtin_amdgcn_raw_ptr_buffer_load_lds(rsx0, dst, 16, off, x0soff, 0, 0);
                else __builtin_amdgcn_raw_ptr_buffer_load_lds(rsx1, dst, 16, off, x1soff, 0, 0);
            }
        }
        mb += TP;
    };

    const int trow = 4 * lq + (l15 >> 2);
    int goff[4];
#pragma unroll
    for (int a = 0; a < 4; ++a) goff[a] = trow * 128 + ((a ^ ((trow >> 1) & 3)) << 5) + (l15 & 3) * 8;
    int xoff[NB];
#pragma unroll
    for (int b = 0; b < NB; ++b) {
        const int ct = wk * NB + b;
        xoff[b] = (SH::WNR + (ct >> 2)) * PLANE + trow * 128 + (((ct & 3) ^ ((trow >> 1) & 3)) << 5) + (l15 & 3) * 8;
    }
    auto compute = [&](int buf) {
        const unsigned char* St = smem + buf * SH::STAGE;
        const unsigned char* Y = St + wc * PLANE;
#pragma unroll
        for (int ks = 0; ks < 2; ++ks) {
            act16x8 yf[4], xf[NB];
#pragma unroll
            for (int a = 0; a < 4; ++a) yf[a] = tr_frag128(Y + ks * 32 * 128 + goff[a]);
#pragma unroll
            for (int b = 0; b < NB; ++b) xf[b] = tr_frag128(St + ks * 32 * 128 + xoff[b]);
#pragma unroll
            for (int a = 0; a < 4; ++a)
#pragma unroll
                for (int b = 0; b < NB; ++b)
                    acc[a][b] = UCLSTM_MFMA_16x16x32(yf[a], xf[b], acc[a][b], 0, 0, 0);
        }
    };

    issue_loads(0);
    __syncthreads();
    for (int step = 0; step < nsteps; ++step) {
        if (step + 1 < nsteps) issue_loads((step + 1) & 1);
        compute(step & 1);
        __syncthreads();
    }

    constexpr int TCc = SH::TC_;
    constexpr int AP = TCc + 4;
    float* At = (float*)smem;
#pragma unroll
    for (int half = 0; half < SH::WNR; ++half) {
        if (wc == half) {
#pragma unroll
            for (int a = 0; a < 4; ++a)
#pragma unroll
                for (int b = 0; b < NB; ++b)
#pragma unroll
                    for (int r = 0; r < 4; ++r) At[(a * 16 + lq * 4 + r) * AP + wk * SH::WCOLS + b * 16 + l15] = acc[a][b][r];
        }
        __syncthreads();
        for (int idx = tid; idx < 64 * TCc; idx += 256) {
            const int pr = idx / TCc, col = idx - pr * TCc;
            const int k = kbase + col;
            const int n = n0 + half * 64 + pr;
            if (k < d.Ktot && n < d.N) {
                float* dst = d.dwp + (long)sp * d.slab + (long)n * d.Ktot + k;
                if (d.slab > 0) *dst = At[pr * AP + col];
                else __hip_atomic_fetch_add(dst, At[pr * AP + col], __ATOMIC_RELAXED, __HIP_MEMORY_SCOPE_AGENT);
            }
        }
        __syncthreads();
    }
#endif
}

constexpr int P3_HALF = 2 * PLANE;
constexpr int P3_BUF = 4 * P3_HALF;
constexpr int P3_SMEM = 2 * P3_BUF;

template <int NSRC, int P3_LEAD>
__global__ __launch_bounds__(512, 1) void igemm_wgrad_p3_kernel(const uclstm_wgrad_desc d, const WDerived dv, const P2 p2) {
#if defined(__HIP_DEVICE_COMPILE__)
    extern __shared__ __attribute__((aligned(16))) unsigned char smem[];
    const int tid = threadIdx.x;
    const int lane = tid & 63;
    const int wave = __builtin_amdgcn_readfirstlane(tid >> 6);
    const int wr = wave >> 2;
    const int wc = wave & 3;
    const int l15 = lane & 15;
    const int lq = lane >> 4;

    const int per_split = dv.n_kt * dv.n_nt;
    const int lid = xcd_remap(blockIdx.x, per_split * d.splits);
    const int sp = lid / per_split;
    const int rr = lid - sp * per_split;
    int nt, kts;
    grouped_tile(rr, dv.n_nt, dv.n_kt, 4, nt, kts);
    int kt = kts;
    if (dv.kt_per_tap > 0) {
        const int ntaps = d.ktap * d.ktap;
        const int cg = kts / ntaps;
        kt = (kts - cg * ntaps) * dv.kt_per_tap + cg;
    }
    const int n0 = nt * 256;
    const int kbase = kt * 256;

    const long m_begin = (long)sp * dv.chunk;
    const long m_end = min(dv.M, m_begin + dv.chunk);
    const int KT = m_begin < dv.M ? (int)((m_end - m_begin) / TP) : 0;
    if (KT == 0) return;
    const int total_halves = 4 * KT;

    const uclstm_seg G = d.seg[0];
    const __amdgpu_buffer_rsrc_t rsy = __builtin_amdgcn_make_buffer_rsrc((void*)G.ptr, 0, p2.ybytes, 0x00020000);
    const __amdgpu_buffer_rsrc_t rsx0 =
        __builtin_amdgcn_make_buffer_rsrc((void*)((const unsigned char*)d.src[0].ptr - p2.xbias[0]), 0, p2.xbytes[0], 0x00020000);
    const __amdgpu_buffer_rsrc_t rsx1 =
        NSRC > 1 ? __builtin_amdgcn_make_buffer_rsrc((void*)((const unsigned char*)d.src[1].ptr - p2.xbias[1]), 0, p2.xbytes[1], 0x00020000)
                 : rsx0;

    const int lrow = lane >> 3;
    const int cp = lane & 7;
    const int sc = 2 * ((cp >> 1) ^ ((lrow >> 1) & 3)) + (cp & 1);
    const int r = 8 * wave + lrow;
    const int Wm = d.W - 1, Hm = d.H - 1;
    const int kseg = dv.kseg0 + dv.kseg1;
    uint32_t yvoff[4], xvoff[4], kxj[4], kyj[4];
    int xsrc[4];
#pragma unroll
    for (int pl = 0; pl < 4; ++pl) {
        const int ny = n0 + pl * 64 + sc * 8;
        const bool yok = ny < d.N && ny >= G.n_begin && ny < G.n_end;
        yvoff[pl] = yok ? (uint32_t)(2 * (r * G.C + G.c_off + (ny - G.n_begin))) : OOB;
        const int k0 = kbase + pl * 64;
        const int xtap = (int)fdiv((uint32_t)k0, dv.dPerTap);
        const int kr = k0 - xtap * kseg;
        const int xs_ = (NSRC > 1 && kr >= dv.kseg0) ? 1 : 0;
        const int xc = (xs_ ? kr - dv.kseg0 : kr) + sc * 8;
        const uclstm_src S = d.src[xs_];
        const bool xok = k0 < d.Ktot && xc < S.C;
        const int tdy = xtap / d.ktap;
        const int ddy = tdy - d.pad;
        const int ddx = (xtap - tdy * d.ktap) - d.pad;
        const int badx = ddx < 0 ? 0 : (ddx > 0 ? Wm : -1);
        const int bady = ddy < 0 ? 0 : (ddy > 0 ? Hm : -1);
        xsrc[pl] = xs_;
        xvoff[pl] = xok ? (uint32_t)(2 * (r * S.C + (ddy * S.Ws + ddx) * S.C + xc) + (int)p2.xbias[xs_]) : OOB;
        if (badx < 0) kxj[pl] = 0xffffffffu;
        else if (d.W >= 64) kxj[pl] = (uint32_t)(badx - r);
        else kxj[pl] = ((r & Wm) == badx) ? 0u : 0xffffffffu;
        kyj[pl] = bady < 0 ? 0xffffffffu : (uint32_t)((bady - (r >> p2.lw)) & Hm);
    }
    const uint32_t ystep = (uint32_t)(2 * G.C), x0step = (uint32_t)(2 * d.src[0].C), x1step = (uint32_t)(2 * d.src[NSRC - 1].C);
    const uint32_t mb0 = (uint32_t)m_begin;

    auto issue_half = [&](int kt_, int slot) {
        unsigned char* dst = smem + (kt_ & 1) * P3_BUF + slot * P3_HALF + wave * 1024;
        const uint32_t mb = mb0 + (uint32_t)kt_ * TP;
        if (slot == 0 || slot == 3) {
            const uint32_t ysoff = mb * ystep;
            const int p0 = slot == 0 ? 0 : 2;
#pragma unroll
            for (int i = 0; i < 2; ++i)
                __builtin_amdgcn_raw_ptr_buffer_load_lds(rsy, (lds_ptr)(dst + i * PLANE), 16, slot == 0 ? yvoff[i] : yvoff[2 + i], ysoff, 0, 0);
            (void)p0;
        } else {
            const uint32_t sy = (mb >> p2.lw) & (uint32_t)Hm;
            const uint32_t sx = mb & (uint32_t)Wm;
            const uint32_t x0soff = mb * x0step, x1soff = mb * x1step;
#pragma unroll
            for (int i = 0; i < 2; ++i) {
                const int pl = (slot == 1 ? 0 : 2) + i;
                const bool ok = (sx != kxj[pl]) & (sy != kyj[pl]);
                const uint32_t off = ok ? xvoff[pl] : OOB;
                if (NSRC == 1 || xsrc[pl] == 0) __builtin_amdgcn_raw_ptr_buffer_load_lds(rsx0, (lds_ptr)(dst + i * PLANE), 16, off, x0soff, 0, 0);
                else __builtin_amdgcn_raw_ptr_buffer_load_lds(rsx1, (lds_ptr)(dst + i * PLANE), 16, off, x1soff, 0, 0);
            }
        }
    };

    f32x4 acc[2][4][2][2];
#pragma unroll
    for (int a = 0; a < 2; ++a)
#pragma unroll
        for (int i = 0; i < 4; ++i)
#pragma unroll
            for (int b = 0; b < 2; ++b)
#pragma unroll
                for (int j = 0; j < 2; ++j) acc[a][i][b][j] = (f32x4){0.f, 0.f, 0.f, 0.f};

    const int trow = 4 * lq + (l15 >> 2);
    const int tsw = (trow >> 1) & 3;
    int goffA[4], goffB[2];
#pragma unroll
    for (int a = 0; a < 4; ++a) goffA[a] = wr * PLANE + trow * 128 + ((a ^ tsw) << 5) + (l15 & 3) * 8;
#pragma unroll
    for (int j = 0; j < 2; ++j) goffB[j] = (wc >> 1) * PLANE + trow * 128 + ((((wc & 1) * 2 + j) ^ tsw) << 5) + (l15 & 3) * 8;

    act16x8 af[4][2], b0f[2][2], b1f[2][2];

#pragma unroll
    for (int q = 0; q < P3_LEAD; ++q)
        if (q < total_halves) issue_half(q >> 2, q & 3);
    if (total_halves >= P3_LEAD) {
        if constexpr (P3_LEAD == 6) asm volatile("s_waitcnt vmcnt(8)" ::: "memory");
        else asm volatile("s_waitcnt vmcnt(10)" ::: "memory");
    } else {
        asm volatile("s_waitcnt vmcnt(0)" ::: "memory");
    }
    if (wr == 1) __builtin_amdgcn_s_barrier();
    __builtin_amdgcn_s_barrier();

    int g = 0;
    for (int ktile = 0; ktile < KT; ++ktile) {
        const unsigned char* base = smem + (ktile & 1) * P3_BUF;
#pragma unroll
        for (int p = 0; p < 4; ++p, ++g) {
            if (p == 0) {
#pragma unroll
                for (int j = 0; j < 2; ++j)
#pragma unroll
                    for (int ks = 0; ks < 2; ++ks) b0f[j][ks] = tr_frag128(base + 1 * P3_HALF + ks * 32 * 128 + goffB[j]);
#pragma unroll
                for (int i = 0; i < 4; ++i)
#pragma unroll
                    for (int ks = 0; ks < 2; ++ks) af[i][ks] = tr_frag128(base + 0 * P3_HALF + ks * 32 * 128 + goffA[i]);
            } else if (p == 1) {
#pragma unroll
                for (int j = 0; j < 2; ++j)
#pragma unroll
                    for (int ks = 0; ks < 2; ++ks) b1f[j][ks] = tr_frag128(base + 2 * P3_HALF + ks * 32 * 128 + goffB[j]);
            } else if (p == 2) {
#pragma unroll
                for (int i = 0; i < 4; ++i)
#pragma unroll
                    for (int ks = 0; ks < 2; ++ks) af[i][ks] = tr_frag128(base + 3 * P3_HALF + ks * 32 * 128 + goffA[i]);
            }
            if (g + P3_LEAD < total_halves) {
                issue_half(ktile + ((p + P3_LEAD) >> 2), (p + P3_LEAD) & 3);
                if constexpr (P3_LEAD == 6) asm volatile("s_waitcnt vmcnt(8)" ::: "memory");
                else asm volatile("s_waitcnt vmcnt(10)" ::: "memory");
            } else {
                asm volatile("s_waitcnt vmcnt(0)" ::: "memory");
            }
            if (P3_LEAD == 7 && p == 0) asm volatile("s_waitcnt lgkmcnt(0)" ::: "memory");
            __builtin_amdgcn_s_barrier();
            asm volatile("s_waitcnt lgkmcnt(0)" ::: "memory");
            __builtin_amdgcn_sched_barrier(0);
            __builtin_amdgcn_s_setprio(1);
            {
                const int mh = (p >= 2) ? 1 : 0;
                const int nh = (p == 1 || p == 2) ? 1 : 0;
#pragma unroll
                for (int ks = 0; ks < 2; ++ks)
#pragma unroll
                    for (int i = 0; i < 4; ++i)
#pragma unroll
                        for (int j = 0; j < 2; ++j) {
                            const act16x8 bb = nh ? b1f[j][ks] : b0f[j][ks];
                            acc[mh][i][nh][j] = UCLSTM_MFMA_16x16x32(af[i][ks], bb, acc[mh][i][nh][j], 0, 0, 0);
                        }
            }
            __builtin_amdgcn_s_setprio(0);
            __builtin_amdgcn_sched_barrier(0);
            __builtin_amdgcn_s_barrier();
        }
    }
    if (wr == 0) __builtin_amdgcn_s_barrier();
    __syncthreads();

    constexpr int AP = 256 + 4;
    float* At = (float*)smem;
#pragma unroll
    for (int pass = 0; pass < 4; ++pass) {
        const int mh = pass >> 1, pwr = pass & 1;
        if (wr == pwr) {
#pragma unroll
            for (int i = 0; i < 4; ++i)
#pragma unroll
                for (int nh = 0; nh < 2; ++nh)
#pragma unroll
                    for (int j = 0; j < 2; ++j)
#pragma unroll
                        for (int q = 0; q < 4; ++q)
                            At[(i * 16 + lq * 4 + q) * AP + nh * 128 + wc * 32 + j * 16 + l15] = mh ? acc[1][i][nh][j][q] : acc[0][i][nh][j][q];
        }
        __syncthreads();
        const int col = tid & 255;
        const int k = kbase + col;
        if (k < d.Ktot) {
            for (int pr = tid >> 8; pr < 64; pr += 2) {
                const int n = n0 + mh * 128 + pwr * 64 + pr;
                if (n < d.N)
                    {
                    float* dst = d.dwp + (long)sp * d.slab + (long)n * d.Ktot + k;
                    if (d.slab > 0) *dst = At[pr * AP + col];
                    else __hip_atomic_fetch_add(dst, At[pr * AP + col], __ATOMIC_RELAXED, __HIP_MEMORY_SCOPE_AGENT);
                }
            }
        }
        __syncthreads();
    }
#endif
}

__device__ __forceinline__ act16x8 tr_frag128_nowait(const unsigned char* __restrict__ p) {
    const short4v lo = __builtin_amdgcn_ds_read_tr16_b64_v4i16((lds_s4p)(p));
    const short4v hi = __builtin_amdgcn_ds_read_tr16_b64_v4i16((lds_s4p)(p + 16 * 128));
    typedef __attribute__((ext_vector_type(8))) short short8v;
    const short8v v = {lo.x, lo.y, lo.z, lo.w, hi.x, hi.y, hi.z, hi.w};
    return __builtin_bit_cast(act16x8, v);
}

template <int NH>
__device__ __forceinline__ void p3w_wait_halves() {
    static_assert(NH == 5 || NH == 6, "vmcnt immediate");
    if constexpr (NH == 6) asm volatile("s_waitcnt vmcnt(24)" ::: "memory");
    else asm volatile("s_waitcnt vmcnt(20)" ::: "memory");
}

template <int NSRC, int LEAD>
__global__ __launch_bounds__(256, 1) void igemm_wgrad_p3w_kernel(const uclstm_wgrad_desc d, const WDerived dv, const P2 p2) {
#if defined(__HIP_DEVICE_COMPILE__)
    static_assert(LEAD == 8 || LEAD == 9, "eight half-tile slots: a half is re-staged one (9) or two (8) phases after its reads");
    extern __shared__ __attribute__((aligned(16))) unsigned char smem[];
    const int tid = threadIdx.x;
    const int lane = tid & 63;
    const int wave = __builtin_amdgcn_readfirstlane(tid >> 6);
    const int wr = wave >> 1;
    const int wc = wave & 1;
    const int l15 = lane & 15;
    const int lq = lane >> 4;

    const int per_split = dv.n_kt * dv.n_nt;
    const int lid = xcd_remap(blockIdx.x, per_split * d.splits);
    const int sp = lid / per_split;
    const int rr = lid - sp * per_split;
    int nt, kts;
    grouped_tile(rr, dv.n_nt, dv.n_kt, 4, nt, kts);
    int kt = kts;
    if (dv.kt_per_tap > 0) {
        const int ntaps = d.ktap * d.ktap;
        const int cg = kts / ntaps;
        kt = (kts - cg * ntaps) * dv.kt_per_tap + cg;
    }
    const int n0 = nt * 256;
    const int kbase = kt * 256;

    const long m_begin = (long)sp * dv.chunk;
    const long m_end = min(dv.M, m_begin + dv.chunk);
    const int KT = m_begin < dv.M ? (int)((m_end - m_begin) / TP) : 0;
    if (KT == 0) return;
    const int total_halves = 4 * KT;

    const uclstm_seg G = d.seg[0];
    const __amdgpu_buffer_rsrc_t rsy = __builtin_amdgcn_make_buffer_rsrc((void*)G.ptr, 0, p2.ybytes, 0x00020000);
    const __amdgpu_buffer_rsrc_t rsx0 =
        __builtin_amdgcn_make_buffer_rsrc((void*)((const unsigned char*)d.src[0].ptr - p2.xbias[0]), 0, p2.xbytes[0], 0x00020000);
    const __amdgpu_buffer_rsrc_t rsx1 =
        NSRC > 1 ? __builtin_amdgcn_make_buffer_rsrc((void*)((const unsigned char*)d.src[1].ptr - p2.xbias[1]), 0, p2.xbytes[1], 0x00020000)
                 : rsx0;

    const int lrow = lane >> 3;
    const int cp = lane & 7;
    const int sc = 2 * ((cp >> 1) ^ ((lrow >> 1) & 3)) + (cp & 1);
    const int r = 8 * wave + lrow;
    const int Wm = d.W - 1, Hm = d.H - 1;
    const int kseg = dv.kseg0 + dv.kseg1;
    uint32_t yvoff[4], xvoff[4], kxj[4], kyj[4];
    int xsrc[4];
#pragma unroll
    for (int pl = 0; pl < 4; ++pl) {
        const int ny = n0 + pl * 64 + sc * 8;
        const bool yok = ny < d.N && ny >= G.n_begin && ny < G.n_end;
        yvoff[pl] = yok ? (uint32_t)(2 * (r * G.C + G.c_off + (ny - G.n_begin))) : OOB;
        const int k0 = kbase + pl * 64;
        const int xtap = (int)fdiv((uint32_t)k0, dv.dPerTap);
        const int kr = k0 - xtap * kseg;
        const int xs_ = (NSRC > 1 && kr >= dv.kseg0) ? 1 : 0;
        const int xc = (xs_ ? kr - dv.kseg0 : kr) + sc * 8;
        const uclstm_src S = d.src[xs_];
        const bool xok = k0 < d.Ktot && xc < S.C;
        const int tdy = xtap / d.ktap;
        const int ddy = tdy - d.pad;
        const int ddx = (xtap - tdy * d.ktap) - d.pad;
        const int badx = ddx < 0 ? 0 : (ddx > 0 ? Wm : -1);
        const int bady = ddy < 0 ? 0 : (ddy > 0 ? Hm : -1);
        xsrc[pl] = xs_;
        xvoff[pl] = xok ? (uint32_t)(2 * (r * S.C + (ddy * S.Ws + ddx) * S.C + xc) + (int)p2.xbias[xs_]) : OOB;
        if (badx < 0) kxj[pl] = 0xffffffffu;
        else if (d.W >= 64) kxj[pl] = (uint32_t)(badx - r);
        else kxj[pl] = ((r & Wm) == badx) ? 0u : 0xffffffffu;
        kyj[pl] = bady < 0 ? 0xffffffffu : (uint32_t)((bady - (r >> p2.lw)) & Hm);
    }
    const uint32_t ystep = (uint32_t)(2 * G.C), x0step = (uint32_t)(2 * d.src[0].C), x1step = (uint32_t)(2 * d.src[NSRC - 1].C);
    const uint32_t mb0 = (uint32_t)m_begin;

    auto issue_half = [&](int kt_, int slot, bool valid) {
        unsigned char* dst = smem + (kt_ & 1) * P3_BUF + slot * P3_HALF + wave * 1024;
#pragma unroll
        for (int hh = 0; hh < 2; ++hh) {
            const uint32_t mb = mb0 + (uint32_t)kt_ * TP + 32u * hh;
            if (slot == 0 || slot == 3) {
                const uint32_t ysoff = mb * ystep;
#pragma unroll
                for (int i = 0; i < 2; ++i)
                    __builtin_amdgcn_raw_ptr_buffer_load_lds(rsy, (lds_ptr)(dst + i * PLANE + hh * 4096), 16, valid ? (slot == 0 ? yvoff[i] : yvoff[2 + i]) : OOB,
                                                             ysoff, 0, 0);
            } else {
                const uint32_t sy = (mb >> p2.lw) & (uint32_t)Hm;
                const uint32_t sx = mb & (uint32_t)Wm;
                const uint32_t x0soff = mb * x0step, x1soff = mb * x1step;
#pragma unroll
                for (int i = 0; i < 2; ++i) {
                    const int pl = (slot == 1 ? 0 : 2) + i;
                    const bool ok = (sx != kxj[pl]) & (sy != kyj[pl]) & valid;
                    const uint32_t off = ok ? xvoff[pl] : OOB;
                    lds_ptr dp = (lds_ptr)(dst + i * PLANE + hh * 4096);
                    const bool s1 = NSRC > 1 && xsrc[pl] != 0;
                    __builtin_amdgcn_raw_ptr_buffer_load_lds(s1 ? rsx1 : rsx0, dp, 16, off, s1 ? x1soff : x0soff, 0, 0);
                }
            }
        }
    };

    f32x4 acc[2][4][2][4];
#pragma unroll
    for (int a = 0; a < 2; ++a)
#pragma unroll
        for (int i = 0; i < 4; ++i)
#pragma unroll
            for (int b = 0; b < 2; ++b)
#pragma unroll
                for (int j = 0; j < 4; ++j) acc[a][i][b][j] = (f32x4){0.f, 0.f, 0.f, 0.f};

    const int trow = 4 * lq + (l15 >> 2);
    const int tsw = (trow >> 1) & 3;
    int goffA[4], goffB[4];
#pragma unroll
    for (int a = 0; a < 4; ++a) {
        goffA[a] = wr * PLANE + trow * 128 + ((a ^ tsw) << 5) + (l15 & 3) * 8;
        goffB[a] = wc * PLANE + trow * 128 + ((a ^ tsw) << 5) + (l15 & 3) * 8;
    }
    act16x8 af[2][4][2], bfr[3][4][2];
    auto read_half = [&](int par, int slot, int bset) {
        const unsigned char* hb = smem + par * P3_BUF + slot * P3_HALF;
        if (slot == 0 || slot == 3) {
#pragma unroll
            for (int i = 0; i < 4; ++i)
#pragma unroll
                for (int ks = 0; ks < 2; ++ks) af[slot == 3][i][ks] = tr_frag128_nowait(hb + ks * 32 * 128 + goffA[i]);
        } else {
#pragma unroll
            for (int j = 0; j < 4; ++j)
#pragma unroll
                for (int ks = 0; ks < 2; ++ks) bfr[bset][j][ks] = tr_frag128_nowait(hb + ks * 32 * 128 + goffB[j]);
        }
    };

#pragma unroll
    for (int q = 0; q < 8; ++q) issue_half(q >> 2, q & 3, q < total_halves);
    p3w_wait_halves<5>();
    __builtin_amdgcn_s_barrier();
    read_half(0, 0, 0);
    read_half(0, 1, 2);
    asm volatile("s_waitcnt lgkmcnt(0)" ::: "memory");
    __builtin_amdgcn_s_barrier();
    if constexpr (LEAD == 9) issue_half(2, 0, 8 < total_halves);

    for (int kt_ = 0; kt_ < KT; ++kt_) {
        const int par = kt_ & 1;
#pragma unroll
        for (int j = 0; j < 4; ++j)
#pragma unroll
            for (int ks = 0; ks < 2; ++ks) bfr[0][j][ks] = bfr[2][j][ks];
#pragma unroll
        for (int q = 0; q < 4; ++q) {
            const int g = 4 * kt_ + q;
            const int mh = q >> 1;
            const int nh = (q == 1 || q == 2) ? 1 : 0;
            __builtin_amdgcn_sched_barrier(0);
            issue_half(kt_ + ((q + LEAD) >> 2), (q + LEAD) & 3, g + LEAD < total_halves);
            __builtin_amdgcn_sched_barrier(0);
            if (q < 2) read_half(par, q + 2, 1);
            else read_half(par ^ 1, q - 2, 2);
#pragma unroll
            for (int ks = 0; ks < 2; ++ks)
#pragma unroll
                for (int i = 0; i < 4; ++i)
#pragma unroll
                    for (int j = 0; j < 4; ++j)
                        acc[mh][i][nh][j] = UCLSTM_MFMA_16x16x32(af[mh][i][ks], bfr[nh][j][ks], acc[mh][i][nh][j], 0, 0, 0);
#pragma unroll
            for (int k = 0; k < 16; ++k) {
                __builtin_amdgcn_sched_group_barrier(0x008, 1, 0);
                __builtin_amdgcn_sched_group_barrier(0x100, 1, 0);
            }
            __builtin_amdgcn_sched_group_barrier(0x008, 16, 0);
            __builtin_amdgcn_sched_barrier(0);
            p3w_wait_halves<LEAD - 3>();
            if constexpr (LEAD == 9) asm volatile("s_waitcnt lgkmcnt(0)" ::: "memory");
            __builtin_amdgcn_s_barrier();
        }
    }
    asm volatile("s_waitcnt vmcnt(0)" ::: "memory");
    __syncthreads();

    constexpr int AP = 256 + 4;
    float* At = (float*)smem;
#pragma unroll
    for (int pass = 0; pass < 4; ++pass) {
        const int mh = pass >> 1, pwr = pass & 1;
        if (wr == pwr) {
#pragma unroll
            for (int i = 0; i < 4; ++i)
#pragma unroll
                for (int nh = 0; nh < 2; ++nh)
#pragma unroll
                    for (int j = 0; j < 4; ++j)
#pragma unroll
                        for (int q = 0; q < 4; ++q)
                            At[(i * 16 + lq * 4 + q) * AP + nh * 128 + wc * 64 + j * 16 + l15] = mh ? acc[1][i][nh][j][q] : acc[0][i][nh][j][q];
        }
        __syncthreads();
        const int k = kbase + tid;
        if (k < d.Ktot) {
            for (int pr = 0; pr < 64; ++pr) {
                const int n = n0 + mh * 128 + pwr * 64 + pr;
                if (n < d.N) {
                    float* dst = d.dwp + (long)sp * d.slab + (long)n * d.Ktot + k;
                    if (d.slab > 0) *dst = At[pr * AP + tid];
                    else __hip_atomic_fetch_add(dst, At[pr * AP + tid], __ATOMIC_RELAXED, __HIP_MEMORY_SCOPE_AGENT);
                }
            }
        }
        __syncthreads();
    }
#endif
}

int auto_splits256(int64_t tiles, int64_t stages, bool slabs, int64_t panel_elems, bool overlapped) {
    const int64_t smax = stages / 8 > 1 ? stages / 8 : 1;
    if (overlapped) {
        static const int min_blocks = [] { const char* e = getenv("UCLSTM_P3_MIN_BLOCKS"); return e ? atoi(e) : 128; }();
        int64_t s = (min_blocks + tiles - 1) / tiles;
        if (s > smax) s = smax;
        return (int)(s < 1 ? 1 : s);
    }
    const double slab_cost = slabs ? (double)panel_elems * 8.0 / 4e12 / 1.9e-6 : 0.0;
    const int64_t fixed = slabs ? 8 : 28;
    int best = 1;
    int64_t best_cost = -1;
    for (int64_t s = 1; s <= smax && tiles * s <= 8192; ++s) {
        const int64_t per = (stages + s - 1) / s;
        const int64_t used = (stages + per - 1) / per;
        const int64_t rounds = (tiles * used + 255) / 256;
        const int64_t cost = rounds * (per + fixed) + (int64_t)(slab_cost * (double)used);
        if (best_cost < 0 || cost < best_cost) {
            best_cost = cost;
            best = (int)s;
        }
    }
    return best;
}

int auto_splits(int64_t tiles, int64_t stages, bool slabs, int64_t panel_elems) {
    const double slab_cost = slabs ? (double)panel_elems * 8.0 / 4e12 / 1.3e-6 : 0.0;
    const int64_t fixed = slabs ? 4 : 8;
    int best = 1;
    int64_t best_cost = -1;
    const int64_t smax = stages / 4 > 1 ? stages / 4 : 1;
    for (int64_t s = 1; s <= smax && tiles * s <= 16384; ++s) {
        const int64_t per = (stages + s - 1) / s;
        const int64_t used = (stages + per - 1) / per;
        const int64_t rounds = (tiles * used + 511) / 512;
        const int64_t cost = rounds * (per + fixed) + (int64_t)(slab_cost * (double)used);
        if (best_cost < 0 || cost < best_cost) {
            best_cost = cost;
            best = (int)s;
        }
    }
    return best;
}

inline bool is_pow2(int v) { return v > 0 && (v & (v - 1)) == 0; }
inline int ilog2(int v) { int l = 0; while ((1 << l) < v) ++l; return l; }


constexpr int WR_PITCH = 72 * 128;
constexpr int WR_SLOTS = 10;
constexpr int WR_RING = WR_SLOTS * WR_PITCH;
constexpr int WR_DZ = 4 * PLANE;
constexpr int WR_SMEM = WR_RING + 2 * WR_DZ;

__global__ __launch_bounds__(256, 1) void igemm_wgrad_c64_kernel(const uclstm_wgrad_desc d, const int src, const int kcol0, const int per_tap,
                                                                  const int tiles_total, const int tiles_per_block, const uint32_t xbytes,
                                                                  const uint32_t ybytes) {
#if defined(__HIP_DEVICE_COMPILE__)
    extern __shared__ __attribute__((aligned(16))) unsigned char smem[];
    unsigned char* Ring = smem;
    unsigned char* Dz = smem + WR_RING;

    const int tid = threadIdx.x;
    const int lane = tid & 63;
    const int wave = __builtin_amdgcn_readfirstlane(tid >> 6);
    const int l15 = lane & 15;
    const int lq = lane >> 4;
    const int H = d.H, W = d.W;
    const int strips = W >> 6;
    const int n_seq = d.n_img * strips;
    const int tiles_per_seq = H >> 2;
    const int t_begin = blockIdx.x * tiles_per_block;
    const int t_end = min(tiles_total, t_begin + tiles_per_block);
    if (t_begin >= t_end) return;

    const uclstm_seg G = d.seg[0];
    const uclstm_src S = d.src[src];
    const __amdgpu_buffer_rsrc_t rsx = __builtin_amdgcn_make_buffer_rsrc((void*)S.ptr, 0, xbytes, 0x00020000);
    const __amdgpu_buffer_rsrc_t rsy = __builtin_amdgcn_make_buffer_rsrc((void*)G.ptr, 0, ybytes, 0x00020000);

    if (strips == 1 && tid < WR_SLOTS * 2 * 8) {
        const int sl = tid >> 4, side = (tid >> 3) & 1, ch = tid & 7;
        *(uint4*)(Ring + sl * WR_PITCH + side * 65 * 128 + ch * 16) = make_uint4(0, 0, 0, 0);
    }

    const int lrow = lane >> 3, cp = lane & 7;
    uint32_t xvoff[2];
#pragma unroll
    for (int i = 0; i < 2; ++i) {
        const int px = 8 * (wave + 4 * i) + lrow;
        const int r = px + 1;
        const int sc = 2 * ((cp >> 1) ^ ((r >> 1) & 3)) + (cp & 1);
        xvoff[i] = (uint32_t)(2 * (px * 64 + sc * 8));
    }
    const int hpos = wave == 0 ? 0 : 65;
    const uint32_t halo_voff = (uint32_t)(2 * ((2 * (((lane & 7) >> 1) ^ ((hpos >> 1) & 3)) + (lane & 1)) * 8));
    uint32_t yvoff[2];
#pragma unroll
    for (int i = 0; i < 2; ++i) {
        const int px = 8 * (wave + 4 * i) + lrow;
        const int sc = 2 * ((cp >> 1) ^ ((px >> 1) & 3)) + (cp & 1);
        yvoff[i] = (uint32_t)(2 * (px * G.C + G.c_off + sc * 8));
    }

    int lk = 0, ly = 0, lslot = 0, loaded = -2, limg = 0, lstrip = 0;
#define WR_ISSUE_NEXT_ROW()                                                                                                 \
    {                                                                                                                       \
        const bool zero_ = ly == H || lk < 0 || lk >= n_seq;                                                                \
        const uint32_t soff_ = zero_ ? 0u : (uint32_t)((limg * H + ly) * W + lstrip * 64) * 128u;                           \
        unsigned char* dst_ = Ring + lslot * WR_PITCH + 128;                                                                \
        __builtin_amdgcn_raw_ptr_buffer_load_lds(rsx, (lds_ptr)(dst_ + wave * 1024), 16, zero_ ? OOB : xvoff[0], soff_, 0, 0);        \
        __builtin_amdgcn_raw_ptr_buffer_load_lds(rsx, (lds_ptr)(dst_ + (wave + 4) * 1024), 16, zero_ ? OOB : xvoff[1], soff_, 0, 0);  \
        if (strips > 1 && wave < 2) {                                                                                       \
            const bool ok_ = !zero_ && (wave == 0 ? lstrip > 0 : lstrip < strips - 1);                                      \
            const uint32_t hs_ = ok_ ? (wave == 0 ? soff_ - 128u : soff_ + 64u * 128u) : 0u;                                \
            if (lane < 8) __builtin_amdgcn_raw_ptr_buffer_load_lds(rsx, (lds_ptr)(Ring + lslot * WR_PITCH + hpos * 128), 16, \
                                                                   ok_ ? halo_voff : OOB, hs_, 0, 0);                       \
        }                                                                                                                   \
        ++loaded;                                                                                                           \
        lslot = lslot == WR_SLOTS - 1 ? 0 : lslot + 1;                                                                      \
        if (ly == H) {                                                                                                      \
            ly = 0;                                                                                                         \
            ++lk;                                                                                                           \
            if (++lstrip == strips) { lstrip = 0; ++limg; }                                                                 \
        } else {                                                                                                            \
            ++ly;                                                                                                           \
        }                                                                                                                   \
    }
#define WR_ISSUE_DZ(k_, tr_, b_)                                                                                            \
    {                                                                                                                       \
        const int img_ = (k_) / strips, st_ = (k_) - img_ * strips;                                                         \
        _Pragma("unroll") for (int pl_ = 0; pl_ < 4; ++pl_) {                                                               \
            const uint32_t so_ = (uint32_t)((img_ * H + 4 * (tr_) + pl_) * W + st_ * 64) * (uint32_t)(2 * G.C);             \
            unsigned char* dp_ = Dz + (b_) * WR_DZ + pl_ * PLANE;                                                           \
            __builtin_amdgcn_raw_ptr_buffer_load_lds(rsy, (lds_ptr)(dp_ + wave * 1024), 16, yvoff[0], so_, 0, 0);           \
            __builtin_amdgcn_raw_ptr_buffer_load_lds(rsy, (lds_ptr)(dp_ + (wave + 4) * 1024), 16, yvoff[1], so_, 0, 0);     \
        }                                                                                                                   \
    }

    const int trow = 4 * lq + (l15 >> 2);
    int yoff[4];
#pragma unroll
    for (int a = 0; a < 4; ++a) yoff[a] = trow * 128 + ((a ^ ((trow >> 1) & 3)) << 5) + (l15 & 3) * 8;
    int xoff[3];
#pragma unroll
    for (int dx = 0; dx < 3; ++dx) {
        const int r = dx + trow;
        xoff[dx] = r * 128 + ((wave ^ ((r >> 1) & 3)) << 5) + (l15 & 3) * 8;
    }

    f32x4 acc[9][4];
#pragma unroll
    for (int t = 0; t < 9; ++t)
#pragma unroll
        for (int a = 0; a < 4; ++a) acc[t][a] = (f32x4){0.f, 0.f, 0.f, 0.f};

    int k = t_begin / tiles_per_seq;
    int tr = t_begin - k * tiles_per_seq;
    WR_ISSUE_DZ(k, tr, 0)
    for (int tt = t_begin; tt < t_end; ++tt) {
        const int v0 = k * (H + 1) + 4 * tr;
        if (tt == t_begin) {
            const int v = v0 - 1;
            if (v < 0) { lk = -1; ly = H; limg = 0; lstrip = -1; } else { lk = v / (H + 1); ly = v - lk * (H + 1); limg = lk / strips; lstrip = lk - limg * strips; }
            lslot = (v + 1) % WR_SLOTS;
            loaded = v - 1;
        }
        if (tt != t_begin && loaded < v0 + 4) __syncthreads();
        while (loaded < v0 + 4) WR_ISSUE_NEXT_ROW()
        asm volatile("s_waitcnt vmcnt(0)" ::: "memory");
        __syncthreads();
        int k1 = k, tr1 = tr + 1;
        if (tr1 == tiles_per_seq) { tr1 = 0; ++k1; }
        if (tt + 1 < t_end) {
            WR_ISSUE_DZ(k1, tr1, (tt + 1 - t_begin) & 1)
            const int upto = min(k1 * (H + 1) + 4 * tr1 + 4, loaded + 4);
            while (loaded < upto) WR_ISSUE_NEXT_ROW()
        }
        const unsigned char* Y = Dz + ((tt - t_begin) & 1) * WR_DZ;
#pragma unroll
        for (int rr = 0; rr < 4; ++rr) {
            const unsigned char* rowp[3];
#pragma unroll
            for (int dy = 0; dy < 3; ++dy) rowp[dy] = Ring + ((v0 + rr + dy) % WR_SLOTS) * WR_PITCH;
#pragma unroll
            for (int ks = 0; ks < 2; ++ks) {
                act16x8 yf[4];
#pragma unroll
                for (int a = 0; a < 4; ++a) yf[a] = tr_frag128(Y + rr * PLANE + ks * 32 * 128 + yoff[a]);
#pragma unroll
                for (int t = 0; t < 9; ++t) {
                    const act16x8 xf = tr_frag128(rowp[t / 3] + ks * 32 * 128 + xoff[t % 3]);
#pragma unroll
                    for (int a = 0; a < 4; ++a) acc[t][a] = UCLSTM_MFMA_16x16x32(yf[a], xf, acc[t][a], 0, 0, 0);
                }
            }
        }
        k = k1;
        tr = tr1;
    }
    float* out = d.dwp + (long)blockIdx.x * d.slab + kcol0 + wave * 16 + l15;
#pragma unroll
    for (int t = 0; t < 9; ++t)
#pragma unroll
        for (int a = 0; a < 4; ++a)
#pragma unroll
            for (int r = 0; r < 4; ++r) {
                const int n = a * 16 + lq * 4 + r;
                if (n < d.N) out[(long)n * d.Ktot + t * per_tap] = acc[t][a][r];
            }
#endif
}
#undef WR_ISSUE_NEXT_ROW
#undef WR_ISSUE_DZ

inline bool wgrad_c64_ok(const uclstm_wgrad_desc& d, bool plain) {
    static const bool off = [] { const char* e = getenv("UCLSTM_WGRAD_RING"); return e && e[0] == '0'; }();
    if (off || !plain || d.ktap != 3 || d.pad != 1 || d.nseg != 1 || d.slab <= 0) return false;
    if (d.N > 64 || d.N <= 0 || (d.W & 63) || (d.H & 3)) return false;
    const uclstm_seg& g = d.seg[0];
    if (g.C != 64 || g.c_off != 0 || g.n_begin != 0) return false;
    for (int s = 0; s < d.nsrc; ++s)
        if (d.src[s].C != 64) return false;
    if (d.Ktot != 9 * 64 * d.nsrc) return false;
    if ((int64_t)d.n_img * d.H * d.W * 128 >= ((int64_t)1 << 31) - (1 << 22)) return false;
    if ((int64_t)d.n_img * (d.W / 64) * (d.H + 1) >= ((int64_t)1 << 30)) return false;
    return true;
}
inline int wgrad_c64_grid(const uclstm_wgrad_desc& d, int& per) {
    const int tiles_total = d.n_img * (d.W / 64) * (d.H / 4);
    const int cap = d.overlapped ? 128 : 256;
    const int blocks = tiles_total < cap ? tiles_total : cap;
    per = (tiles_total + blocks - 1) / blocks;
    return (tiles_total + per - 1) / per;
}

template <int WN, int NSRC>
int32_t launch_p2(const uclstm_wgrad_desc& d, const WDerived& dv, const P2& p2, int64_t nblk, hipStream_t st) {
    static bool attr_done = false;
    if (!attr_done) {
        (void)hipFuncSetAttribute((const void*)igemm_wgrad_p2_kernel<WN, NSRC>, hipFuncAttributeMaxDynamicSharedMemorySize,
                                   WShape<WN>::SMEM);
        attr_done = true;
    }
    UCLSTM_LAUNCH((igemm_wgrad_p2_kernel<WN, NSRC>), dim3((unsigned)nblk), dim3(256), WShape<WN>::SMEM, st, d, dv, p2);
    return UCLSTM_OK;
}

bool wsrc_ok(const uclstm_src& s) {
    return s.ptr && s.C > 0 && (s.C % 8) == 0 && s.Hs > 0 && s.Ws > 0 && ((uintptr_t)s.ptr % 16) == 0;
}

}

namespace {
int32_t wgrad_run(const uclstm_wgrad_desc* dp, void* stream, int query) {
    const bool plan_only = query != 0;
    if (!dp) return UCLSTM_E_BADARG;
    const uclstm_wgrad_desc& d = *dp;
    if (d.n_img <= 0 || d.H <= 0 || d.W <= 0) return UCLSTM_E_BADARG;
    if (d.ktap < 1 || d.ktap > 7 || d.scale < 1 || d.scale > 2 || d.pad < 0 || d.pad > 3) return UCLSTM_E_BADARG;
    if (d.nsrc < 1 || d.nsrc > 2 || (!d.dwp && !plan_only) || d.N <= 0 || (d.N % 8) || d.splits < 0 || d.slab < 0) return UCLSTM_E_BADARG;
    if (d.slab > 0 && d.slab < (int64_t)d.N * d.Ktot) return UCLSTM_E_BADARG;
    if (d.nseg < 1 || d.nseg > 4) return UCLSTM_E_BADARG;
    bool plain = d.scale == 1;
    for (int s = 0; s < d.nsrc; ++s) {
        if (!wsrc_ok(d.src[s])) return UCLSTM_E_BADARG;
        if ((int64_t)d.n_img * d.src[s].Hs * d.src[s].Ws * d.src[s].C >= ((int64_t)1 << 31) - (1 << 20)) return UCLSTM_E_BADARG;
        plain = plain && d.src[s].Hs == d.H && d.src[s].Ws == d.W && d.src[s].offY == 0 && d.src[s].offX == 0;
    }
    for (int i = 0; i < d.nseg; ++i) {
        const uclstm_seg& sg = d.seg[i];
        if (!sg.ptr || (sg.n_begin % 8) || (sg.n_end % 8) || sg.n_end <= sg.n_begin || (sg.C % 8) || (sg.c_off % 8) ||
            sg.c_off + (sg.n_end - sg.n_begin) > sg.C || sg.Hd <= 0 || sg.Wd <= 0 || sg.scale < 1 || ((uintptr_t)sg.ptr % 16))
            return UCLSTM_E_BADARG;
        if ((int64_t)d.n_img * sg.Hd * sg.Wd * sg.C >= ((int64_t)1 << 31) - (1 << 20)) return UCLSTM_E_BADARG;
        plain = plain && sg.scale == 1 && sg.oy == 0 && sg.ox == 0 && sg.Hd == d.H && sg.Wd == d.W;
    }
    WDerived dv;
    dv.kseg0 = round_up32(d.src[0].C, 64);
    dv.kseg1 = d.nsrc > 1 ? round_up32(d.src[1].C, 64) : 0;
    const int taps = d.ktap * d.ktap;
    if (d.Ktot != taps * (dv.kseg0 + dv.kseg1)) return UCLSTM_E_BADARG;
    if (wgrad_c64_ok(d, plain)) {
        int per = 0;
        const int grid = wgrad_c64_grid(d, per);
        if (query == 2) return 4;
        if (query == 1) return grid;
        if (d.splits != grid) return UCLSTM_E_BADARG;
        static bool attr_r = false;
        if (!attr_r) {
            (void)hipFuncSetAttribute((const void*)igemm_wgrad_c64_kernel, hipFuncAttributeMaxDynamicSharedMemorySize, WR_SMEM);
            attr_r = true;
        }
        const int tiles_total = d.n_img * (d.W / 64) * (d.H / 4);
        const uint32_t ybytes = (uint32_t)((int64_t)d.n_img * d.H * d.W * d.seg[0].C * 2);
        for (int sidx = 0; sidx < d.nsrc; ++sidx) {
            const uint32_t xbytes = (uint32_t)((int64_t)d.n_img * d.H * d.W * 128);
            UCLSTM_LAUNCH(igemm_wgrad_c64_kernel, dim3(grid), dim3(256), WR_SMEM, (hipStream_t)stream, d, sidx, sidx * 64, 64 * d.nsrc, tiles_total,
                          per, xbytes, ybytes);
        }
        return UCLSTM_OK;
    }
    dv.M = (long)d.n_img * d.H * d.W;
    if (dv.M >= ((long)1 << 31) - 4096) return UCLSTM_E_BADARG;
    dv.dHW = make_fastdiv((uint32_t)(d.H * d.W));
    dv.dW = make_fastdiv((uint32_t)d.W);
    dv.dPerTap = make_fastdiv((uint32_t)(dv.kseg0 + dv.kseg1));

    static const bool no_fast = [] { const char* e = getenv("UCLSTM_WGRAD_GENERIC"); return e && e[0] == '1'; }();
    bool fast = plain && !no_fast && d.nseg == 1 && is_pow2(d.H) && is_pow2(d.W) && (dv.M % TP) == 0 &&
                ((d.ktap == 3 && d.pad == 1) || (d.ktap == 1 && d.pad == 0));
    P2 p2{};
    if (fast) {
        const int64_t lim = ((int64_t)1 << 31) - (1 << 22);
        const int64_t yb = dv.M * d.seg[0].C * 2;
        fast = yb < lim;
        p2.ybytes = (uint32_t)yb;
        for (int s = 0; s < d.nsrc && fast; ++s) {
            const int64_t bias = (int64_t)(d.src[s].Ws + 1) * d.src[s].C * 2;
            const int64_t xb = dv.M * d.src[s].C * 2 + bias;
            fast = xb < lim;
            p2.xbias[s] = (uint32_t)bias;
            p2.xbytes[s] = (uint32_t)xb;
        }
        p2.lw = ilog2(d.W);
        p2.lh = ilog2(d.H);
    }
    static const bool no_p3 = [] { const char* e = getenv("UCLSTM_WGRAD_NO256"); return e && e[0] == '1'; }();
    const bool big = fast && !no_p3 && d.N >= 256;
    static const bool no_192 = [] { const char* e = getenv("UCLSTM_WGRAD_NO192"); return e && e[0] == '1'; }();
    const int wn = (fast && d.N <= 64) ? ((!no_192 && d.Ktot % 192 == 0) ? 3 : 1) : 2;
    const int tn = big ? 256 : (wn == 2 ? 128 : 64), tc = big ? 256 : (wn == 2 ? 128 : (wn == 3 ? 192 : 256));
    dv.n_kt = (d.Ktot + tc - 1) / tc;
    dv.n_nt = (d.N + tn - 1) / tn;
    dv.kt_per_tap = (fast && ((dv.kseg0 + dv.kseg1) % tc) == 0) ? (dv.kseg0 + dv.kseg1) / tc : 0;
    uclstm_wgrad_desc dd = d;
    const bool slabs = d.slab > 0;
    if (dd.splits <= 0)
        dd.splits = big ? auto_splits256((int64_t)dv.n_kt * dv.n_nt, (dv.M + TP - 1) / TP, slabs, (int64_t)d.N * d.Ktot, d.overlapped != 0)
                        : auto_splits((int64_t)dv.n_kt * dv.n_nt, (dv.M + TP - 1) / TP, slabs, (int64_t)d.N * d.Ktot);
    long chunk = (dv.M + dd.splits - 1) / dd.splits;
    chunk = (chunk + TP - 1) / TP * TP;
    dv.chunk = chunk;
    dd.splits = (int)((dv.M + chunk - 1) / chunk);
    if (query == 2) return big ? 3 : (fast ? (wn == 2 ? 2 : 1) : 0);
    if (plan_only) return dd.splits;
    const int64_t nblk = (int64_t)dv.n_kt * dv.n_nt * dd.splits;
    if (nblk <= 0 || nblk > 0x7fffffff) return UCLSTM_E_BADARG;
    hipStream_t st = (hipStream_t)stream;

    if (big) {
        static bool attr3 = false;
        static const bool lead7 = [] { const char* e = getenv("UCLSTM_P3_LEAD"); return !(e && e[0] == '6'); }();
        if (!attr3) {
            (void)hipFuncSetAttribute((const void*)igemm_wgrad_p3_kernel<1, 6>, hipFuncAttributeMaxDynamicSharedMemorySize, P3_SMEM);
            (void)hipFuncSetAttribute((const void*)igemm_wgrad_p3_kernel<2, 6>, hipFuncAttributeMaxDynamicSharedMemorySize, P3_SMEM);
            (void)hipFuncSetAttribute((const void*)igemm_wgrad_p3_kernel<1, 7>, hipFuncAttributeMaxDynamicSharedMemorySize, P3_SMEM);
            (void)hipFuncSetAttribute((const void*)igemm_wgrad_p3_kernel<2, 7>, hipFuncAttributeMaxDynamicSharedMemorySize, P3_SMEM);
            (void)hipFuncSetAttribute((const void*)igemm_wgrad_p3w_kernel<1, 8>, hipFuncAttributeMaxDynamicSharedMemorySize, P3_SMEM);
            (void)hipFuncSetAttribute((const void*)igemm_wgrad_p3w_kernel<2, 8>, hipFuncAttributeMaxDynamicSharedMemorySize, P3_SMEM);
            (void)hipFuncSetAttribute((const void*)igemm_wgrad_p3w_kernel<1, 9>, hipFuncAttributeMaxDynamicSharedMemorySize, P3_SMEM);
            (void)hipFuncSetAttribute((const void*)igemm_wgrad_p3w_kernel<2, 9>, hipFuncAttributeMaxDynamicSharedMemorySize, P3_SMEM);
            attr3 = true;
        }
        static const bool waves8 = [] { const char* e = getenv("UCLSTM_P3_WAVES"); return e && e[0] == '8'; }();
        if (!waves8) {
            if (lead7) {
                if (d.nsrc == 1) UCLSTM_LAUNCH((igemm_wgrad_p3w_kernel<1, 9>), dim3((unsigned)nblk), dim3(256), P3_SMEM, st, dd, dv, p2);
                else UCLSTM_LAUNCH((igemm_wgrad_p3w_kernel<2, 9>), dim3((unsigned)nblk), dim3(256), P3_SMEM, st, dd, dv, p2);
            } else {
                if (d.nsrc == 1) UCLSTM_LAUNCH((igemm_wgrad_p3w_kernel<1, 8>), dim3((unsigned)nblk), dim3(256), P3_SMEM, st, dd, dv, p2);
                else UCLSTM_LAUNCH((igemm_wgrad_p3w_kernel<2, 8>), dim3((unsigned)nblk), dim3(256), P3_SMEM, st, dd, dv, p2);
            }
            return UCLSTM_OK;
        }
        if (lead7) {
            if (d.nsrc == 1) UCLSTM_LAUNCH((igemm_wgrad_p3_kernel<1, 7>), dim3((unsigned)nblk), dim3(512), P3_SMEM, st, dd, dv, p2);
            else UCLSTM_LAUNCH((igemm_wgrad_p3_kernel<2, 7>), dim3((unsigned)nblk), dim3(512), P3_SMEM, st, dd, dv, p2);
        } else {
            if (d.nsrc == 1) UCLSTM_LAUNCH((igemm_wgrad_p3_kernel<1, 6>), dim3((unsigned)nblk), dim3(512), P3_SMEM, st, dd, dv, p2);
            else UCLSTM_LAUNCH((igemm_wgrad_p3_kernel<2, 6>), dim3((unsigned)nblk), dim3(512), P3_SMEM, st, dd, dv, p2);
        }
        return UCLSTM_OK;
    }
    if (fast) {
        if (wn == 1) return d.nsrc == 1 ? launch_p2<1, 1>(dd, dv, p2, nblk, st) : launch_p2<1, 2>(dd, dv, p2, nblk, st);
        if (wn == 3) return d.nsrc == 1 ? launch_p2<3, 1>(dd, dv, p2, nblk, st) : launch_p2<3, 2>(dd, dv, p2, nblk, st);
        return d.nsrc == 1 ? launch_p2<2, 1>(dd, dv, p2, nblk, st) : launch_p2<2, 2>(dd, dv, p2, nblk, st);
    }
    static bool attr_done = false;
    if (!attr_done) {
        (void)hipFuncSetAttribute((const void*)igemm_wgrad_kernel<true>, hipFuncAttributeMaxDynamicSharedMemorySize, SMEM_BYTES);
        (void)hipFuncSetAttribute((const void*)igemm_wgrad_kernel<false>, hipFuncAttributeMaxDynamicSharedMemorySize, SMEM_BYTES);
        attr_done = true;
    }
    if (plain)
        UCLSTM_LAUNCH(igemm_wgrad_kernel<true>, dim3((unsigned)nblk), dim3(256), SMEM_BYTES, st, dd, dv);
    else
        UCLSTM_LAUNCH(igemm_wgrad_kernel<false>, dim3((unsigned)nblk), dim3(256), SMEM_BYTES, st, dd, dv);
    return UCLSTM_OK;
}
}

extern "C" int32_t uclstm_igemm_wgrad(const uclstm_wgrad_desc* d, void* stream) { return wgrad_run(d, stream, 0); }

#ifndef UCLSTM_ACT_F16
extern "C" int32_t uclstm_igemm_wgrad_splits(const uclstm_wgrad_desc* d) { return wgrad_run(d, nullptr, 1); }
#endif
#ifndef UCLSTM_ACT_F16
extern "C" int32_t uclstm_igemm_wgrad_shape(const uclstm_wgrad_desc* d) { return wgrad_run(d, nullptr, 2); }
#endif
```

Baseline: 19980 frames/s.

## Walk only valid pixels per tap in 3x3 wgrad p3 kernels

Adds a valid-pixel walk mode to the pipelined wgrad kernels. For each 3x3 tap, the M dimension is restricted to output pixels whose shifted input lies inside the image, so border rows and columns that would be zero contributions are skipped instead of masked. The per-row pixel index is computed with magic division and interleaved into the MFMA schedule so it hides behind compute. The split heuristic is also updated to cost per-tap stage counts. The trade-off is extra integer address arithmetic, more template instantiations, and uneven tile lengths across taps.

```diff
diff --git a/include/uclstm.h b/include/uclstm.h
--- a/include/uclstm.h
+++ b/include/uclstm.h
@@ -94,6 +94,7 @@
 int32_t uclstm_igemm_wgrad(const uclstm_wgrad_desc* d, void* stream);
 int32_t uclstm_igemm_wgrad_splits(const uclstm_wgrad_desc* d);
 int32_t uclstm_igemm_wgrad_shape(const uclstm_wgrad_desc* d);
+int64_t uclstm_igemm_wgrad_walk(const uclstm_wgrad_desc* d, int32_t tap, int64_t i0, int32_t n, int32_t* pixels);
 
 #define UCLSTM_NMODE_IDENTITY 0
 #define UCLSTM_NMODE_LSTM     1
diff --git a/unet-convlstm_amd/_lib.py b/unet-convlstm_amd/_lib.py
--- a/unet-convlstm_amd/_lib.py
+++ b/unet-convlstm_amd/_lib.py
@@ -145,6 +145,7 @@
     "uclstm_igemm_wgrad": [C.POINTER(WgradDesc), _P],
     "uclstm_igemm_wgrad_splits": [C.POINTER(WgradDesc)],
     "uclstm_igemm_wgrad_shape": [C.POINTER(WgradDesc)],
+    "uclstm_igemm_wgrad_walk": [C.POINTER(WgradDesc), _I, _L, _I, C.POINTER(C.c_int32)],
     "uclstm_pack_weights": [C.POINTER(PackDesc), _P, _P, _P],
     "uclstm_pack_job_init": [C.POINTER(PackJob), C.POINTER(PackDesc), _P, _P, _I],
     "uclstm_pack_weights_batched": [_P, _I, _I, _I, _P],
@@ -254,7 +255,7 @@
     "uclstm_source_hash": [],
     "uclstm_last_error_string": [],
 }
-_RESTYPES = {"uclstm_build_arch": C.c_char_p, "uclstm_source_hash": C.c_char_p, "uclstm_last_error_string": C.c_char_p, "uclstm_bn_bwd_reduce_rows": C.c_int64, "uclstm_bn_pool_bwd_rows": C.c_int64,
+_RESTYPES = {"uclstm_igemm_wgrad_walk": C.c_int64, "uclstm_build_arch": C.c_char_p, "uclstm_source_hash": C.c_char_p, "uclstm_last_error_string": C.c_char_p, "uclstm_bn_bwd_reduce_rows": C.c_int64, "uclstm_bn_pool_bwd_rows": C.c_int64,
              "uclstm_eval_stats_rows": C.c_int64, "uclstm_colsum_ordered_rows": C.c_int64, "uclstm_outconv_bwd_ordered_rows": C.c_int64, "uclstm_head3x3_bwd_ordered_rows": C.c_int64,
              "uclstm_loss_fwd_ordered_rows": C.c_int64, "uclstm_sumsq_ordered_rows": C.c_int64, "uclstm_metric_sums_ordered_rows": C.c_int64, "uclstm_metric_sums_vec_rows": C.c_int64,
              "uclstm_bn_add_relu_bwd_rows": C.c_int64, "uclstm_select_workspace_bytes": C.c_int64}
diff --git a/unet-convlstm_amd/csrc/igemm_wgrad.hip b/unet-convlstm_amd/csrc/igemm_wgrad.hip
--- a/unet-convlstm_amd/csrc/igemm_wgrad.hip
+++ b/unet-convlstm_amd/csrc/igemm_wgrad.hip
@@ -1,4 +1,5 @@
 #include "common.h"
+#include "wgrad_walk.h"
 #include <cstdlib>
 
 namespace {
@@ -20,6 +21,7 @@
     long chunk;
     int kt_per_tap;
     FastDiv dHW, dW, dPerTap;
+    WalkDiv dWv[2], dNv[2][2];
 };
 
 typedef __attribute__((address_space(3))) short4v* lds_s4p;
@@ -420,7 +422,31 @@
 constexpr int P3_BUF = 4 * P3_HALF;
 constexpr int P3_SMEM = 2 * P3_BUF;
 
-template <int NSRC, int P3_LEAD>
+struct WalkTile {
+    ValidWalk w;
+    uint32_t i0;
+    int KT;
+    int kt;
+    int ddy, ddx;
+};
+__device__ __forceinline__ WalkTile walk_tile(const uclstm_wgrad_desc& d, const WDerived& dv, int kts, int sp) {
+    WalkTile t;
+    const int cg = kts / 9;
+    const int tap = (int)((0x862075314ull >> (4 * (kts - cg * 9))) & 15);
+    t.kt = tap * dv.kt_per_tap + cg;
+    const int ty = tap / 3;
+    t.ddy = ty - 1;
+    t.ddx = tap - 3 * ty - 1;
+    const int iy = t.ddy != 0, ix = t.ddx != 0;
+    t.w = make_valid_walk(d.n_img, d.H, d.W, t.ddy, t.ddx, dv.dNv[iy][ix], dv.dWv[ix]);
+    int kb;
+    valid_walk_range(t.w.total, d.splits, sp, kb, t.KT);
+    t.i0 = (uint32_t)kb * TP;
+    t.w.total = min(t.w.total, (uint32_t)(kb + t.KT) * TP);
+    return t;
+}
+
+template <int NSRC, int P3_LEAD, bool VW>
 __global__ __launch_bounds__(512, 1) void igemm_wgrad_p3_kernel(const uclstm_wgrad_desc d, const WDerived dv, const P2 p2) {
 #if defined(__HIP_DEVICE_COMPILE__)
     extern __shared__ __attribute__((aligned(16))) unsigned char smem[];
@@ -439,18 +465,23 @@
     int nt, kts;
     grouped_tile(rr, dv.n_nt, dv.n_kt, 4, nt, kts);
     int kt = kts;
-    if (dv.kt_per_tap > 0) {
+    if (!VW && dv.kt_per_tap > 0) {
         const int ntaps = d.ktap * d.ktap;
         const int cg = kts / ntaps;
         kt = (kts - cg * ntaps) * dv.kt_per_tap + cg;
     }
+    WalkTile wt{};
+    if constexpr (VW) {
+        wt = walk_tile(d, dv, kts, sp);
+        kt = wt.kt;
+    }
     const int n0 = nt * 256;
     const int kbase = kt * 256;
 
     const long m_begin = (long)sp * dv.chunk;
     const long m_end = min(dv.M, m_begin + dv.chunk);
-    const int KT = m_begin < dv.M ? (int)((m_end - m_begin) / TP) : 0;
-    if (KT == 0) return;
+    const int KT = VW ? wt.KT : (m_begin < dv.M ? (int)((m_end - m_begin) / TP) : 0);
+    if (KT == 0 && !(VW && d.slab > 0)) return;
     const int total_halves = 4 * KT;
 
     const uclstm_seg G = d.seg[0];
@@ -465,6 +496,7 @@
     const int cp = lane & 7;
     const int sc = 2 * ((cp >> 1) ^ ((lrow >> 1) & 3)) + (cp & 1);
     const int r = 8 * wave + lrow;
+    const int rv = VW ? 0 : r;
     const int Wm = d.W - 1, Hm = d.H - 1;
     const int kseg = dv.kseg0 + dv.kseg1;
     uint32_t yvoff[4], xvoff[4], kxj[4], kyj[4];
@@ -473,7 +505,7 @@
     for (int pl = 0; pl < 4; ++pl) {
         const int ny = n0 + pl * 64 + sc * 8;
         const bool yok = ny < d.N && ny >= G.n_begin && ny < G.n_end;
-        yvoff[pl] = yok ? (uint32_t)(2 * (r * G.C + G.c_off + (ny - G.n_begin))) : OOB;
+        yvoff[pl] = yok ? (uint32_t)(2 * (rv * G.C + G.c_off + (ny - G.n_begin))) : OOB;
         const int k0 = kbase + pl * 64;
         const int xtap = (int)fdiv((uint32_t)k0, dv.dPerTap);
         const int kr = k0 - xtap * kseg;
@@ -487,7 +519,7 @@
         const int badx = ddx < 0 ? 0 : (ddx > 0 ? Wm : -1);
         const int bady = ddy < 0 ? 0 : (ddy > 0 ? Hm : -1);
         xsrc[pl] = xs_;
-        xvoff[pl] = xok ? (uint32_t)(2 * (r * S.C + (ddy * S.Ws + ddx) * S.C + xc) + (int)p2.xbias[xs_]) : OOB;
+        xvoff[pl] = xok ? (uint32_t)(2 * (rv * S.C + (ddy * S.Ws + ddx) * S.C + xc) + (int)p2.xbias[xs_]) : OOB;
         if (badx < 0) kxj[pl] = 0xffffffffu;
         else if (d.W >= 64) kxj[pl] = (uint32_t)(badx - r);
         else kxj[pl] = ((r & Wm) == badx) ? 0u : 0xffffffffu;
@@ -498,6 +530,24 @@
 
     auto issue_half = [&](int kt_, int slot) {
         unsigned char* dst = smem + (kt_ & 1) * P3_BUF + slot * P3_HALF + wave * 1024;
+        if constexpr (VW) {
+            const uint32_t pix = valid_walk_pixel<true>(wt.w, wt.i0 + (uint32_t)kt_ * TP + (uint32_t)r);
+            const uint32_t none = pix == WALK_NONE ? OOB : 0u;
+#pragma unroll
+            for (int i = 0; i < 2; ++i) {
+                lds_ptr dp = (lds_ptr)(dst + i * PLANE);
+                if (slot == 0 || slot == 3) {
+                    const uint32_t pb = walk_mul<true>(pix, ystep) | none;
+                    __builtin_amdgcn_raw_ptr_buffer_load_lds(rsy, dp, 16, __builtin_elementwise_add_sat(pb, yvoff[(slot == 0 ? 0 : 2) + i]), 0, 0, 0);
+                } else {
+                    const int pl = (slot == 1 ? 0 : 2) + i;
+                    const bool s1 = NSRC > 1 && xsrc[pl] != 0;
+                    const uint32_t pb = walk_mul<true>(pix, s1 ? x1step : x0step) | none;
+                    __builtin_amdgcn_raw_ptr_buffer_load_lds(s1 ? rsx1 : rsx0, dp, 16, __builtin_elementwise_add_sat(pb, xvoff[pl]), 0, 0, 0);
+                }
+            }
+            return;
+        }
         const uint32_t mb = mb0 + (uint32_t)kt_ * TP;
         if (slot == 0 || slot == 3) {
             const uint32_t ysoff = mb * ystep;
@@ -661,7 +711,7 @@
     else asm volatile("s_waitcnt vmcnt(20)" ::: "memory");
 }
 
-template <int NSRC, int LEAD>
+template <int NSRC, int LEAD, bool VW>
 __global__ __launch_bounds__(256, 1) void igemm_wgrad_p3w_kernel(const uclstm_wgrad_desc d, const WDerived dv, const P2 p2) {
 #if defined(__HIP_DEVICE_COMPILE__)
     static_assert(LEAD == 8 || LEAD == 9, "eight half-tile slots: a half is re-staged one (9) or two (8) phases after its reads");
@@ -681,18 +731,23 @@
     int nt, kts;
     grouped_tile(rr, dv.n_nt, dv.n_kt, 4, nt, kts);
     int kt = kts;
-    if (dv.kt_per_tap > 0) {
+    if (!VW && dv.kt_per_tap > 0) {
         const int ntaps = d.ktap * d.ktap;
         const int cg = kts / ntaps;
         kt = (kts - cg * ntaps) * dv.kt_per_tap + cg;
     }
+    WalkTile wt{};
+    if constexpr (VW) {
+        wt = walk_tile(d, dv, kts, sp);
+        kt = wt.kt;
+    }
     const int n0 = nt * 256;
     const int kbase = kt * 256;
 
     const long m_begin = (long)sp * dv.chunk;
     const long m_end = min(dv.M, m_begin + dv.chunk);
-    const int KT = m_begin < dv.M ? (int)((m_end - m_begin) / TP) : 0;
-    if (KT == 0) return;
+    const int KT = VW ? wt.KT : (m_begin < dv.M ? (int)((m_end - m_begin) / TP) : 0);
+    if (KT == 0 && !(VW && d.slab > 0)) return;
     const int total_halves = 4 * KT;
 
     const uclstm_seg G = d.seg[0];
@@ -707,6 +762,7 @@
     const int cp = lane & 7;
     const int sc = 2 * ((cp >> 1) ^ ((lrow >> 1) & 3)) + (cp & 1);
     const int r = 8 * wave + lrow;
+    const int rv = VW ? 0 : r;
     const int Wm = d.W - 1, Hm = d.H - 1;
     const int kseg = dv.kseg0 + dv.kseg1;
     uint32_t yvoff[4], xvoff[4], kxj[4], kyj[4];
@@ -715,7 +771,7 @@
     for (int pl = 0; pl < 4; ++pl) {
         const int ny = n0 + pl * 64 + sc * 8;
         const bool yok = ny < d.N && ny >= G.n_begin && ny < G.n_end;
-        yvoff[pl] = yok ? (uint32_t)(2 * (r * G.C + G.c_off + (ny - G.n_begin))) : OOB;
+        yvoff[pl] = yok ? (uint32_t)(2 * (rv * G.C + G.c_off + (ny - G.n_begin))) : OOB;
         const int k0 = kbase + pl * 64;
         const int xtap = (int)fdiv((uint32_t)k0, dv.dPerTap);
         const int kr = k0 - xtap * kseg;
@@ -729,7 +785,7 @@
         const int badx = ddx < 0 ? 0 : (ddx > 0 ? Wm : -1);
         const int bady = ddy < 0 ? 0 : (ddy > 0 ? Hm : -1);
         xsrc[pl] = xs_;
-        xvoff[pl] = xok ? (uint32_t)(2 * (r * S.C + (ddy * S.Ws + ddx) * S.C + xc) + (int)p2.xbias[xs_]) : OOB;
+        xvoff[pl] = xok ? (uint32_t)(2 * (rv * S.C + (ddy * S.Ws + ddx) * S.C + xc) + (int)p2.xbias[xs_]) : OOB;
         if (badx < 0) kxj[pl] = 0xffffffffu;
         else if (d.W >= 64) kxj[pl] = (uint32_t)(badx - r);
         else kxj[pl] = ((r & Wm) == badx) ? 0u : 0xffffffffu;
@@ -738,8 +794,64 @@
     const uint32_t ystep = (uint32_t)(2 * G.C), x0step = (uint32_t)(2 * d.src[0].C), x1step = (uint32_t)(2 * d.src[NSRC - 1].C);
     const uint32_t mb0 = (uint32_t)m_begin;
 
+    constexpr int WALK_STEPS = 14;
+    uint32_t pby[2] = {OOB, OOB}, pbx0[2] = {OOB, OOB}, pbx1[2] = {OOB, OOB};
+    uint32_t wq[2] = {0, 0}, wimg[2] = {0, 0}, wj[2] = {0, 0}, wpix[2] = {0, 0};
+    auto walk_step = [&](int kt_, int step) {
+        const int hh = step / 7, st = step - 7 * hh;
+        const ValidWalk& w = wt.w;
+        const uint32_t i = wt.i0 + (uint32_t)kt_ * TP + 32u * hh + (uint32_t)r;
+        if (st == 0) {
+            wq[hh] = walk_div_hi(i, w.dNv);
+            asm volatile("" : "+v"(wq[hh]));
+        } else if (st == 1) {
+            wimg[hh] = wq[hh] >> w.dNv.shift;
+            wj[hh] = walk_in_image<true>(w, i, wimg[hh]);
+            asm volatile("" : "+v"(wj[hh]));
+        } else if (st == 2) {
+            wq[hh] = walk_div_hi(wj[hh], w.dWv);
+            asm volatile("" : "+v"(wq[hh]));
+        } else if (st == 3) {
+            const uint32_t yy = wq[hh] >> w.dWv.shift;
+            wpix[hh] = walk_compose<true>(w, i, wimg[hh], yy, walk_in_row<true>(w, wj[hh], yy));
+            asm volatile("" : "+v"(wpix[hh]));
+        } else {
+            const uint32_t none = wpix[hh] == WALK_NONE ? OOB : 0u;
+            if (st == 4) {
+                pby[hh] = walk_mul<true>(wpix[hh], ystep) | none;
+                asm volatile("" : "+v"(pby[hh]));
+            } else if (st == 5) {
+                pbx0[hh] = walk_mul<true>(wpix[hh], x0step) | none;
+                asm volatile("" : "+v"(pbx0[hh]));
+            } else if (NSRC > 1) {
+                pbx1[hh] = walk_mul<true>(wpix[hh], x1step) | none;
+                asm volatile("" : "+v"(pbx1[hh]));
+            }
+        }
+    };
+    auto walk_ktile = [&](int kt_) {
+#pragma unroll
+        for (int step = 0; step < WALK_STEPS; ++step) walk_step(kt_, step);
+    };
     auto issue_half = [&](int kt_, int slot, bool valid) {
         unsigned char* dst = smem + (kt_ & 1) * P3_BUF + slot * P3_HALF + wave * 1024;
+        if constexpr (VW) {
+#pragma unroll
+            for (int hh = 0; hh < 2; ++hh)
+#pragma unroll
+                for (int i = 0; i < 2; ++i) {
+                    lds_ptr dp = (lds_ptr)(dst + i * PLANE + hh * 4096);
+                    if (slot == 0 || slot == 3) {
+                        __builtin_amdgcn_raw_ptr_buffer_load_lds(rsy, dp, 16, __builtin_elementwise_add_sat(pby[hh], yvoff[(slot == 0 ? 0 : 2) + i]), 0, 0, 0);
+                    } else {
+                        const int pl = (slot == 1 ? 0 : 2) + i;
+                        const bool s1 = NSRC > 1 && xsrc[pl] != 0;
+                        __builtin_amdgcn_raw_ptr_buffer_load_lds(s1 ? rsx1 : rsx0, dp, 16, __builtin_elementwise_add_sat(s1 ? pbx1[hh] : pbx0[hh], xvoff[pl]),
+                                                                 0, 0, 0);
+                    }
+                }
+            return;
+        }
 #pragma unroll
         for (int hh = 0; hh < 2; ++hh) {
             const uint32_t mb = mb0 + (uint32_t)kt_ * TP + 32u * hh;
@@ -801,7 +913,11 @@
     };
 
 #pragma unroll
-    for (int q = 0; q < 8; ++q) issue_half(q >> 2, q & 3, q < total_halves);
+    for (int q = 0; q < 8; ++q) {
+        if (VW && (q & 3) == 0) walk_ktile(q >> 2);
+        issue_half(q >> 2, q & 3, q < total_halves);
+    }
+    if constexpr (VW) walk_ktile(2);
     p3w_wait_halves<5>();
     __builtin_amdgcn_s_barrier();
     read_half(0, 0, 0);
@@ -826,19 +942,40 @@
             __builtin_amdgcn_sched_barrier(0);
             if (q < 2) read_half(par, q + 2, 1);
             else read_half(par ^ 1, q - 2, 2);
-#pragma unroll
-            for (int ks = 0; ks < 2; ++ks)
+            const bool walk_phase = VW && q == (LEAD == 9 ? 2 : 3);
+#pragma unroll
+            for (int ks = 0; ks < 2; ++ks) {
+                if (walk_phase && ks == 1) {
+#pragma unroll
+                    for (int k = 0; k < 16; ++k) {
+                        __builtin_amdgcn_sched_group_barrier(0x008, 1, 0);
+                        __builtin_amdgcn_sched_group_barrier(0x100, 1, 0);
+                    }
+                    __builtin_amdgcn_sched_barrier(0);
+#pragma unroll
+                    for (int i = 0; i < 4; ++i)
+#pragma unroll
+                        for (int j = 0; j < 4; ++j) {
+                            acc[mh][i][nh][j] = UCLSTM_MFMA_16x16x32(af[mh][i][ks], bfr[nh][j][ks], acc[mh][i][nh][j], 0, 0, 0);
+                            if (4 * i + j < WALK_STEPS) walk_step(kt_ + 3, 4 * i + j);
+                            __builtin_amdgcn_sched_barrier(0);
+                        }
+                    break;
+                }
 #pragma unroll
                 for (int i = 0; i < 4; ++i)
 #pragma unroll
                     for (int j = 0; j < 4; ++j)
                         acc[mh][i][nh][j] = UCLSTM_MFMA_16x16x32(af[mh][i][ks], bfr[nh][j][ks], acc[mh][i][nh][j], 0, 0, 0);
-#pragma unroll
-            for (int k = 0; k < 16; ++k) {
-                __builtin_amdgcn_sched_group_barrier(0x008, 1, 0);
-                __builtin_amdgcn_sched_group_barrier(0x100, 1, 0);
-            }
-            __builtin_amdgcn_sched_group_barrier(0x008, 16, 0);
+            }
+            if (!walk_phase) {
+#pragma unroll
+                for (int k = 0; k < 16; ++k) {
+                    __builtin_amdgcn_sched_group_barrier(0x008, 1, 0);
+                    __builtin_amdgcn_sched_group_barrier(0x100, 1, 0);
+                }
+                __builtin_amdgcn_sched_group_barrier(0x008, 16, 0);
+            }
             __builtin_amdgcn_sched_barrier(0);
             p3w_wait_halves<LEAD - 3>();
             if constexpr (LEAD == 9) asm volatile("s_waitcnt lgkmcnt(0)" ::: "memory");
@@ -881,7 +1018,7 @@
 #endif
 }
 
-int auto_splits256(int64_t tiles, int64_t stages, bool slabs, int64_t panel_elems, bool overlapped) {
+int auto_splits256(int64_t tiles, int64_t stages, bool slabs, int64_t panel_elems, bool overlapped, const int64_t* tap_stages) {
     const int64_t smax = stages / 8 > 1 ? stages / 8 : 1;
     if (overlapped) {
         static const int min_blocks = [] { const char* e = getenv("UCLSTM_P3_MIN_BLOCKS"); return e ? atoi(e) : 128; }();
@@ -897,7 +1034,12 @@
         const int64_t per = (stages + s - 1) / s;
         const int64_t used = (stages + per - 1) / per;
         const int64_t rounds = (tiles * used + 255) / 256;
-        const int64_t cost = rounds * (per + fixed) + (int64_t)(slab_cost * (double)used);
+        int64_t cost = rounds * (per + fixed) + (int64_t)(slab_cost * (double)used);
+        if (tap_stages) {
+            int64_t sum = 0;
+            for (int t = 0; t < 9; ++t) sum += (tap_stages[t] + used - 1) / used;
+            cost = (int64_t)((double)rounds * ((double)sum / 9.0 + (double)fixed) + slab_cost * (double)used);
+        }
         if (best_cost < 0 || cost < best_cost) {
             best_cost = cost;
             best = (int)s;
@@ -1217,10 +1359,24 @@
     dv.n_kt = (d.Ktot + tc - 1) / tc;
     dv.n_nt = (d.N + tn - 1) / tn;
     dv.kt_per_tap = (fast && ((dv.kseg0 + dv.kseg1) % tc) == 0) ? (dv.kseg0 + dv.kseg1) / tc : 0;
+    static const bool no_vw = [] { const char* e = getenv("UCLSTM_WGRAD_VALID"); return e && e[0] == '0'; }();
+    const bool vw = big && !no_vw && dv.kt_per_tap > 0 && d.ktap == 3 && d.pad == 1 && dv.M < ((long)1 << 24) - 4096;
+    for (int iy = 0; iy < 2; ++iy)
+        for (int ix = 0; ix < 2; ++ix) {
+            const int hv = d.H - iy > 0 ? d.H - iy : 0, wv = d.W - ix > 0 ? d.W - ix : 0;
+            dv.dWv[ix] = make_walkdiv((uint32_t)wv);
+            dv.dNv[iy][ix] = make_walkdiv((uint32_t)(hv * wv));
+        }
     uclstm_wgrad_desc dd = d;
     const bool slabs = d.slab > 0;
+    int64_t tap_stages[9];
+    for (int t = 0; t < 9; ++t) {
+        const int hv = d.H - (t / 3 != 1) > 0 ? d.H - (t / 3 != 1) : 0, wv = d.W - (t % 3 != 1) > 0 ? d.W - (t % 3 != 1) : 0;
+        tap_stages[t] = ((int64_t)d.n_img * hv * wv + TP - 1) / TP;
+    }
     if (dd.splits <= 0)
-        dd.splits = big ? auto_splits256((int64_t)dv.n_kt * dv.n_nt, (dv.M + TP - 1) / TP, slabs, (int64_t)d.N * d.Ktot, d.overlapped != 0)
+        dd.splits = big ? auto_splits256((int64_t)dv.n_kt * dv.n_nt, (dv.M + TP - 1) / TP, slabs, (int64_t)d.N * d.Ktot, d.overlapped != 0,
+                                         vw ? tap_stages : nullptr)
                         : auto_splits((int64_t)dv.n_kt * dv.n_nt, (dv.M + TP - 1) / TP, slabs, (int64_t)d.N * d.Ktot);
     long chunk = (dv.M + dd.splits - 1) / dd.splits;
     chunk = (chunk + TP - 1) / TP * TP;
@@ -1233,38 +1389,34 @@
     hipStream_t st = (hipStream_t)stream;
 
     if (big) {
-        static bool attr3 = false;
         static const bool lead7 = [] { const char* e = getenv("UCLSTM_P3_LEAD"); return !(e && e[0] == '6'); }();
-        if (!attr3) {
-            (void)hipFuncSetAttribute((const void*)igemm_wgrad_p3_kernel<1, 6>, hipFuncAttributeMaxDynamicSharedMemorySize, P3_SMEM);
-            (void)hipFuncSetAttribute((const void*)igemm_wgrad_p3_kernel<2, 6>, hipFuncAttributeMaxDynamicSharedMemorySize, P3_SMEM);
-            (void)hipFuncSetAttribute((const void*)igemm_wgrad_p3_kernel<1, 7>, hipFuncAttributeMaxDynamicSharedMemorySize, P3_SMEM);
-            (void)hipFuncSetAttribute((const void*)igemm_wgrad_p3_kernel<2, 7>, hipFuncAttributeMaxDynamicSharedMemorySize, P3_SMEM);
-            (void)hipFuncSetAttribute((const void*)igemm_wgrad_p3w_kernel<1, 8>, hipFuncAttributeMaxDynamicSharedMemorySize, P3_SMEM);
-            (void)hipFuncSetAttribute((const void*)igemm_wgrad_p3w_kernel<2, 8>, hipFuncAttributeMaxDynamicSharedMemorySize, P3_SMEM);
-            (void)hipFuncSetAttribute((const void*)igemm_wgrad_p3w_kernel<1, 9>, hipFuncAttributeMaxDynamicSharedMemorySize, P3_SMEM);
-            (void)hipFuncSetAttribute((const void*)igemm_wgrad_p3w_kernel<2, 9>, hipFuncAttributeMaxDynamicSharedMemorySize, P3_SMEM);
-            attr3 = true;
-        }
         static const bool waves8 = [] { const char* e = getenv("UCLSTM_P3_WAVES"); return e && e[0] == '8'; }();
-        if (!waves8) {
-            if (lead7) {
-                if (d.nsrc == 1) UCLSTM_LAUNCH((igemm_wgrad_p3w_kernel<1, 9>), dim3((unsigned)nblk), dim3(256), P3_SMEM, st, dd, dv, p2);
-                else UCLSTM_LAUNCH((igemm_wgrad_p3w_kernel<2, 9>), dim3((unsigned)nblk), dim3(256), P3_SMEM, st, dd, dv, p2);
-            } else {
-                if (d.nsrc == 1) UCLSTM_LAUNCH((igemm_wgrad_p3w_kernel<1, 8>), dim3((unsigned)nblk), dim3(256), P3_SMEM, st, dd, dv, p2);
-                else UCLSTM_LAUNCH((igemm_wgrad_p3w_kernel<2, 8>), dim3((unsigned)nblk), dim3(256), P3_SMEM, st, dd, dv, p2);
-            }
-            return UCLSTM_OK;
-        }
-        if (lead7) {
-            if (d.nsrc == 1) UCLSTM_LAUNCH((igemm_wgrad_p3_kernel<1, 7>), dim3((unsigned)nblk), dim3(512), P3_SMEM, st, dd, dv, p2);
-            else UCLSTM_LAUNCH((igemm_wgrad_p3_kernel<2, 7>), dim3((unsigned)nblk), dim3(512), P3_SMEM, st, dd, dv, p2);
-        } else {
-            if (d.nsrc == 1) UCLSTM_LAUNCH((igemm_wgrad_p3_kernel<1, 6>), dim3((unsigned)nblk), dim3(512), P3_SMEM, st, dd, dv, p2);
-            else UCLSTM_LAUNCH((igemm_wgrad_p3_kernel<2, 6>), dim3((unsigned)nblk), dim3(512), P3_SMEM, st, dd, dv, p2);
-        }
-        return UCLSTM_OK;
+        const dim3 grid((unsigned)nblk);
+#define P3_GO(KERNEL, THREADS)                                                                                              \
+    {                                                                                                                       \
+        static bool attr_ = false;                                                                                          \
+        if (!attr_) {                                                                                                       \
+            (void)hipFuncSetAttribute((const void*)KERNEL, hipFuncAttributeMaxDynamicSharedMemorySize, P3_SMEM);            \
+            attr_ = true;                                                                                                   \
+        }                                                                                                                   \
+        UCLSTM_LAUNCH((KERNEL), grid, dim3(THREADS), P3_SMEM, st, dd, dv, p2);                                               \
+        return UCLSTM_OK;                                                                                                   \
+    }
+#define P3_PICK(NAME, DEEP, SHALLOW, THREADS)                                                                               \
+    {                                                                                                                       \
+        if (lead7 && d.nsrc == 1 && vw) P3_GO((NAME<1, DEEP, true>), THREADS)                                                \
+        if (lead7 && d.nsrc == 1) P3_GO((NAME<1, DEEP, false>), THREADS)                                                     \
+        if (lead7 && vw) P3_GO((NAME<2, DEEP, true>), THREADS)                                                               \
+        if (lead7) P3_GO((NAME<2, DEEP, false>), THREADS)                                                                    \
+        if (d.nsrc == 1 && vw) P3_GO((NAME<1, SHALLOW, true>), THREADS)                                                      \
+        if (d.nsrc == 1) P3_GO((NAME<1, SHALLOW, false>), THREADS)                                                           \
+        if (vw) P3_GO((NAME<2, SHALLOW, true>), THREADS)                                                                     \
+        P3_GO((NAME<2, SHALLOW, false>), THREADS)                                                                            \
+    }
+        if (!waves8) P3_PICK(igemm_wgrad_p3w_kernel, 9, 8, 256)
+        P3_PICK(igemm_wgrad_p3_kernel, 7, 6, 512)
+#undef P3_PICK
+#undef P3_GO
     }
     if (fast) {
         if (wn == 1) return d.nsrc == 1 ? launch_p2<1, 1>(dd, dv, p2, nblk, st) : launch_p2<1, 2>(dd, dv, p2, nblk, st);
@@ -1293,3 +1445,21 @@
 #ifndef UCLSTM_ACT_F16
 extern "C" int32_t uclstm_igemm_wgrad_shape(const uclstm_wgrad_desc* d) { return wgrad_run(d, nullptr, 2); }
 #endif
+#ifndef UCLSTM_ACT_F16
+extern "C" int64_t uclstm_igemm_wgrad_walk(const uclstm_wgrad_desc* d, int32_t tap, int64_t i0, int32_t n, int32_t* pixels) {
+    if (!d || d->n_img <= 0 || d->H <= 0 || d->W <= 0 || d->ktap < 1 || d->ktap > 7 || d->pad < 0 || d->pad > 3) return UCLSTM_E_BADARG;
+    if (tap < 0 || tap >= d->ktap * d->ktap || i0 < 0 || n < 0 || (n > 0 && !pixels)) return UCLSTM_E_BADARG;
+    if ((int64_t)d->n_img * d->H * d->W >= ((int64_t)1 << 31) - 4096 || i0 + n >= ((int64_t)1 << 31)) return UCLSTM_E_BADARG;
+    const int ty = tap / d->ktap;
+    const int ddy = ty - d->pad, ddx = tap - ty * d->ktap - d->pad;
+    const int ay = ddy < 0 ? -ddy : ddy, ax = ddx < 0 ? -ddx : ddx;
+    const int hv = d->H > ay ? d->H - ay : 0, wv = d->W > ax ? d->W - ax : 0;
+    const ValidWalk w = make_valid_walk(d->n_img, d->H, d->W, ddy, ddx, make_walkdiv((uint32_t)(hv * wv)), make_walkdiv((uint32_t)wv));
+    const bool small = valid_walk_small(w, d->n_img);
+    for (int32_t k = 0; k < n; ++k) {
+        const uint32_t p = small ? valid_walk_pixel<true>(w, (uint32_t)(i0 + k)) : valid_walk_pixel<false>(w, (uint32_t)(i0 + k));
+        pixels[k] = p == WALK_NONE ? -1 : (int32_t)p;
+    }
+    return (int64_t)w.total;
+}
+#endif
diff --git a/unet-convlstm_amd/csrc/wgrad_walk.h b/unet-convlstm_amd/csrc/wgrad_walk.h
--- /dev/null
+++ b/unet-convlstm_amd/csrc/wgrad_walk.h
@@ -0,0 +1,104 @@
+#pragma once
+#include "common.h"
+
+constexpr uint32_t WALK_NONE = 0xffffffffu;
+
+struct WalkDiv {
+    uint32_t magic, shift;
+};
+static inline WalkDiv make_walkdiv(uint32_t d) {
+    if (d < 1) d = 1;
+    uint32_t l = 0;
+    while ((1ull << l) < d) ++l;
+    WalkDiv f;
+    f.magic = (uint32_t)(((1ull << (31 + l)) + d - 1) / d);
+    f.shift = l;
+    return f;
+}
+__host__ __device__ inline uint32_t walk_div_hi(uint32_t m, const WalkDiv& f) {
+#if defined(__HIP_DEVICE_COMPILE__)
+    return __umulhi(m << 1, f.magic);
+#else
+    return (uint32_t)(((uint64_t)(m << 1) * f.magic) >> 32);
+#endif
+}
+__host__ __device__ inline uint32_t walk_div(uint32_t m, const WalkDiv& f) { return walk_div_hi(m, f) >> f.shift; }
+
+template <bool SMALL>
+__host__ __device__ inline uint32_t walk_mul(uint32_t a, uint32_t b) {
+    if constexpr (SMALL) {
+#if defined(__HIP_DEVICE_COMPILE__)
+        return __umul24(a, b);
+#else
+        return (a & 0xffffffu) * (b & 0xffffffu);
+#endif
+    } else {
+        return a * b;
+    }
+}
+
+struct ValidWalk {
+    int32_t y0, x0, hv, wv;
+    int32_t nv;
+    int32_t HW, W;
+    int32_t lHW, lW;
+    uint32_t total;
+    WalkDiv dNv, dWv;
+};
+
+__host__ __device__ inline ValidWalk make_valid_walk(int n_img, int H, int W, int ddy, int ddx, const WalkDiv& dNv, const WalkDiv& dWv) {
+    ValidWalk w;
+    const int ay = ddy < 0 ? -ddy : ddy, ax = ddx < 0 ? -ddx : ddx;
+    w.y0 = ddy < 0 ? ay : 0;
+    w.x0 = ddx < 0 ? ax : 0;
+    w.hv = H > ay ? H - ay : 0;
+    w.wv = W > ax ? W - ax : 0;
+    w.nv = w.hv * w.wv;
+    w.HW = H * W;
+    w.W = W;
+    w.lW = w.lHW = -1;
+    if ((H & (H - 1)) == 0 && (W & (W - 1)) == 0) {
+        int lw = 0, lh = 0;
+        while ((1 << lw) < W) ++lw;
+        while ((1 << lh) < H) ++lh;
+        w.lW = lw;
+        w.lHW = lw + lh;
+    }
+    w.total = (uint32_t)n_img * (uint32_t)w.nv;
+    w.dNv = dNv;
+    w.dWv = dWv;
+    return w;
+}
+__host__ __device__ inline bool valid_walk_small(const ValidWalk& w, int n_img) {
+    return w.lW >= 0 && (int64_t)n_img * w.HW < ((int64_t)1 << 24);
+}
+
+template <bool SMALL>
+__host__ __device__ inline uint32_t walk_in_image(const ValidWalk& w, uint32_t i, uint32_t img) { return i - walk_mul<SMALL>(img, (uint32_t)w.nv); }
+template <bool SMALL>
+__host__ __device__ inline uint32_t walk_in_row(const ValidWalk& w, uint32_t j, uint32_t yy) { return j - walk_mul<SMALL>(yy, (uint32_t)w.wv); }
+template <bool SMALL>
+__host__ __device__ inline uint32_t walk_compose(const ValidWalk& w, uint32_t i, uint32_t img, uint32_t yy, uint32_t xx) {
+    uint32_t p;
+    if constexpr (SMALL) p = (img << w.lHW) + (((uint32_t)w.y0 + yy) << w.lW) + (uint32_t)w.x0 + xx;
+    else p = img * (uint32_t)w.HW + ((uint32_t)w.y0 + yy) * (uint32_t)w.W + (uint32_t)w.x0 + xx;
+    return i < w.total ? p : WALK_NONE;
+}
+
+template <bool SMALL>
+__host__ __device__ inline uint32_t valid_walk_pixel(const ValidWalk& w, uint32_t i) {
+    const uint32_t img = walk_div(i, w.dNv);
+    const uint32_t j = walk_in_image<SMALL>(w, i, img);
+    const uint32_t yy = walk_div(j, w.dWv);
+    const uint32_t xx = walk_in_row<SMALL>(w, j, yy);
+    return walk_compose<SMALL>(w, i, img, yy, xx);
+}
+
+__host__ __device__ inline int valid_walk_ktiles(uint32_t total) { return (int)((total + 63u) >> 6); }
+__host__ __device__ inline void valid_walk_range(uint32_t total, int splits, int sp, int& kb, int& kt) {
+    const int n = valid_walk_ktiles(total);
+    const int per = (n + splits - 1) / splits;
+    kb = sp * per;
+    kt = n - kb < per ? n - kb : per;
+    if (kt < 0) kt = 0;
+}
```

Result: faster. 20610 frames/s (median of 6 runs) (+3.1%).
